# arkworks-rs/ripp

Hardware: AMD Instinct MI355X
Metric: SIPP prover pairing-products/sec at n=2^20 BLS12-381 (higher is better)
Workload: dtype u32

## Files before the change

### ripp_amd/csrc/engine.hip

```cpp
#include <hip/hip_runtime.h>
#include <atomic>
#include <csignal>
#include <sched.h>
#include <condition_variable>
#include <deque>
#include <functional>
#include <memory>
#include <future>
#include <chrono>
#include <cmath>
#include <cstdio>
#include <cstring>
#include <cstdlib>
#include <mutex>
#include <string>
#include <thread>
#include <vector>
#ifndef RIPP_BUILD_STAMP
#define RIPP_BUILD_STAMP __DATE__ " " __TIME__
#endif
#include "../../include/ripp_hip.h"
#include "kernels.hpp"
#include "line_products.hpp"
#include "msm.hpp"
// ... 36 lines not shown
        auto task = std::make_shared<std::packaged_task<decltype(f())()>>(std::forward<F>(f));
        auto fut = task->get_future();
        push([task]() { (*task)(); });
        return fut;
    }
    void set_hot(bool h) { hot_.store(h, std::memory_order_release); }
    template <class F> void parallel(int n, F&& fn) {
        if (n <= 0) return;
        std::atomic<int> left{n - 1};
        for (int t = 1; t < n; ++t) push([&fn, &left, t]() { fn(t); left.fetch_sub(1, std::memory_order_release); });
        fn(0);
        while (left.load(std::memory_order_acquire) > 0) RIPP_CPU_RELAX();
    }
private:
    void push(std::function<void()> job) {
        { std::lock_guard<std::mutex> lk(mu_); q_.emplace_back(std::move(job)); }
        pending_.fetch_add(1, std::memory_order_release);
        if (sleepers_.load(std::memory_order_acquire) > 0) cv_.notify_one();
    }
    void run() {
        for (;;) {
            std::function<void()> job;
            const auto t0 = std::chrono::steady_clock::now();
            for (int spin = 0; hot_.load(std::memory_order_acquire) && pending_.load(std::memory_order_acquire) == 0; ++spin) {
                RIPP_CPU_RELAX();
                if ((spin & 1023) == 1023 && std::chrono::steady_clock::now() - t0 > std::chrono::milliseconds(50)) break;
            }
            {
                std::unique_lock<std::mutex> lk(mu_);
                if (q_.empty()) { sleepers_.fetch_add(1); cv_.wait(lk, [this]() { return stop_ || !q_.empty(); }); sleepers_.fetch_sub(1); }
                if (stop_ && q_.empty()) return;
                job = std::move(q_.front()); q_.pop_front();
                pending_.fetch_sub(1, std::memory_order_release);
            }
            job();
        }
    }
    std::vector<std::thread> th_; std::deque<std::function<void()>> q_; std::mutex mu_; std::condition_variable cv_; bool stop_ = false;
    std::atomic<int> pending_{0}, sleepers_{0}; std::atomic<bool> hot_{false};
};
static int effective_cpus();
HostPool& host_pool() {
    static HostPool pool([]() -> unsigned { if (const char* s = std::getenv("RIPP_HOST_WORKERS")) { const int v = std::atoi(s); if (v >= 1 && v <= 64) return (unsigned)v; } return effective_cpus() >= 14 ? 11u : 6u; }());
    return pool;
}
static int effective_cpus() {
    static const int n = []() {
        int c = (int)std::thread::hardware_concurrency();
        cpu_set_t set; CPU_ZERO(&set);
        if (sched_getaffinity(0, sizeof set, &set) == 0) { const int a = CPU_COUNT(&set); if (a > 0) c = a; }
        if (FILE* f = std::fopen("/sys/fs/cgroup/cpu.max", "r")) {
            char q[32] = {0}; long period = 0;
            if (std::fscanf(f, "%31s %ld", q, &period) == 2 && period > 0 && q[0] != 'm') { const long quota = std::atol(q); if (quota > 0) c = std::min<long>(c, (quota + period - 1) / period); }
            std::fclose(f);
        }
        return std::max(1, c);
    }();
    return n;
}
static bool hot_workers_pay(int ranks_on_node) { return effective_cpus() / std::max(1, ranks_on_node) >= 8; }
double now_ms(); bool trace_on();
void pairing_values(const Fp12* rows, int count, Fp12* out, int parts = 0) {
    if (parts <= 0) parts = host_pool().size() >= 11 ? (count >= 2 ? 5 : 8) : (count >= 2 ? 3 : 4);
    struct Seg { int k, hi, lo; };
    std::vector<Seg> segs;
    for (int k = 0; k < count; ++k) for (int g = 0; g < parts; ++g) segs.push_back({k, 62 - (63 * g) / parts, 62 - (63 * (g + 1)) / parts + 1});
    std::vector<Fp12> E(segs.size());
    auto work = [&rows, &segs, &E](size_t t) { const Seg& sg = segs[t]; E[t] = final_exponentiation(miller_combine_range(rows + (size_t)sg.k * N_LINES, sg.hi, sg.lo)); };
    const double tp0 = now_ms();
    host_pool().parallel((int)segs.size(), [&work](int t) { work((size_t)t); });
    const double tp1 = now_ms();
    host_pool().parallel(count, [&](int k) {
        Fp12 c = E[(size_t)k * parts];
        for (int g = 1; g < parts; ++g) { const Seg& sg = segs[(size_t)k * parts + g]; for (int b = sg.hi; b >= sg.lo; --b) c = cyclotomic_sqr(c); c = mul(c, E[(size_t)k * parts + g]); }
        out[k] = BLS_X_NEG ? conj(c) : c; });
    if (trace_on()) fprintf(stderr, "[ripp] pairing_values(%d x %d): ranges %.3f ms, join %.3f ms\n", count, parts, tp1 - tp0, now_ms() - tp1);
}
struct Engine;
Engine* g_engine = nullptr;
std::atomic<int> g_live_handles{0};

#define HIPCHK(expr) do { hipError_t e_ = (expr); if (e_ != hipSuccess) { set_err(std::string(#expr) + ": " + hipGetErrorString(e_)); return RIPP_ERR_DEVICE; } } while (0)
void set_err(const std::string& s) { g_err = s; }
bool trace_on();
double now_ms() { return std::chrono::duration<double, std::milli>(std::chrono::steady_clock::now().time_since_epoch()).count(); }

inline unsigned nblk(size_t n, unsigned b) { return (unsigned)((n + b - 1) / b); }
inline uint32_t pow2_floor(uint32_t v) { uint32_t p = 1; while ((p << 1) <= v && (p << 1) != 0) p <<= 1; return p; }

std::atomic<size_t> g_dev_bytes{0};
std::atomic<uint64_t> g_call_epoch{1};
struct Engine;
thread_local Engine* t_engine = nullptr;
size_t evict_idle_scratch(Engine* e);
struct DevBuf {
    void* p = nullptr; size_t cap = 0; uint64_t epoch = 0;
    int32_t reserve(size_t bytes) {
        epoch = g_call_epoch.load(std::memory_order_relaxed);
        if (bytes <= cap) return RIPP_OK;
        release();
        hipError_t err = hipMalloc(&p, bytes);
        if (err == hipErrorOutOfMemory && t_engine) {
            (void)hipGetLastError();
            const size_t freed = evict_idle_scratch(t_engine);
            if (trace_on()) fprintf(stderr, "[ripp] out of device memory for %zu bytes: %zu bytes of idle scratch freed, retrying\n", bytes, freed);
            err = freed ? hipMalloc(&p, bytes) : err;
        }
        if (err != hipSuccess) { p = nullptr; (void)hipGetLastError(); set_err(std::string("hipMalloc(&p, bytes): ") + hipGetErrorString(err) + " (" + std::to_string(bytes) + " bytes wanted, " + std::to_string(g_dev_bytes.load()) + " held by the library)"); return RIPP_ERR_DEVICE; }
        cap = bytes; g_dev_bytes.fetch_add(bytes, std::memory_order_relaxed); return RIPP_OK;
    }
    void release() { if (p) { (void)hipFree(p); g_dev_bytes.fetch_sub(cap, std::memory_order_relaxed); } p = nullptr; cap = 0; }
    template <class T> T* as() { return reinterpret_cast<T*>(p); }
};

struct PinBuf {
    void* p = nullptr; size_t cap = 0; hipEvent_t ev = nullptr; bool pending = false;
    bool blocking = false;
    bool ev_blocking = false;
    int32_t wait() { if (pending) { HIPCHK(hipEventSynchronize(ev)); pending = false; } return RIPP_OK; }
    int32_t reserve(size_t bytes) {
        int32_t rc = wait(); if (rc) return rc;
        if (ev && ev_blocking != blocking) { (void)hipEventDestroy(ev); ev = nullptr; }
        if (!ev) { HIPCHK(hipEventCreateWithFlags(&ev, hipEventDisableTiming | (blocking ? hipEventBlockingSync : 0))); ev_blocking = blocking; }
        if (bytes <= cap) return RIPP_OK;
        if (p) { (void)hipHostFree(p); p = nullptr; cap = 0; }
        HIPCHK(hipHostMalloc(&p, bytes, hipHostMallocDefault)); cap = bytes; return RIPP_OK;
    }
    int32_t send(void* dst, size_t bytes, hipStream_t st) {
        HIPCHK(hipMemcpyAsync(dst, p, bytes, hipMemcpyHostToDevice, st)); HIPCHK(hipEventRecord(ev, st)); pending = true; return RIPP_OK;
    }
    void release() { if (pending && ev) (void)hipEventSynchronize(ev); pending = false; if (p) (void)hipHostFree(p); p = nullptr; cap = 0; if (ev) (void)hipEventDestroy(ev); ev = nullptr; }
    template <class T> T* as() { return reinterpret_cast<T*>(p); }
};

struct MsmScratch {
    DevBuf digits, hist, offs, cursor, slotoffs, spw, sorted, slots, buckets, seg, seg2, win, out;
    DevBuf ext;
    DevBuf flags;
    DevBuf nflag;
    void* host_out = nullptr;
    void release() { for (DevBuf* b : {&digits, &hist, &offs, &cursor, &slotoffs, &spw, &sorted, &slots, &buckets, &seg, &seg2, &win, &out, &ext, &flags, &nflag}) b->release(); if (host_out) (void)hipHostFree(host_out); host_out = nullptr; }
};

struct Timer {
    hipEvent_t a{}, b{};
    int32_t init() { HIPCHK(hipEventCreate(&a)); HIPCHK(hipEventCreate(&b)); return RIPP_OK; }
    void destroy() { if (a) (void)hipEventDestroy(a); if (b) (void)hipEventDestroy(b); a = b = nullptr; }
};

struct Engine {
    int device = -1;
    hipStream_t stream = nullptr, stream2 = nullptr;
    hipEvent_t ev_fork = nullptr, ev_join = nullptr, ev_join3 = nullptr;
    hipEvent_t ev_t0 = nullptr, ev_t1 = nullptr;
    int n_simd = 1024;
    DevBuf lines, partA, partB, jacG1, jacG2, tmpA, tmpB, tmpR, affG1, affG2;
    DevBuf qtab;
    MsmScratch msm_scratch[2];
    DevBuf kzg_q[2];
    PinBuf stage[4];
    DevBuf kzg_bases[2];
    hipStream_t stream3 = nullptr;
    hipStream_t stream4 = nullptr;
    hipEvent_t ev_join4 = nullptr;
    DevBuf fold_tab1, fold_mult, fold_tab, fold_jac1, fold_jac2;
    DevBuf fix_flags, scale_flags;
    const void* tab_owner = nullptr;
    struct JobBufCache { DevBuf d[15]; PinBuf p[4]; bool full = false; void release() { for (DevBuf& b : d) b.release(); for (PinBuf& b : p) b.release(); full = false; } } job_cache;
    size_t msm_chunk_min = (size_t)1 << 20;
    size_t msm_lds_sort_min = 0;
    const void* g2tab_hi = nullptr; size_t g2tab_half = 0;
    size_t vm_scale_max = (size_t)1 << 14;
    size_t vm_joint_max = (size_t)1 << 13;
    size_t lp_fq_min = 0;
    size_t ml_fq_min = 0;
    size_t fq_min_g1 = (size_t)1 << 12;
    size_t fq_min = (size_t)1 << 15;
    size_t fold_tab_min = 32768;
    size_t msm_vm_merge_max = 16384;
    hipStream_t stream5 = nullptr;
    hipEvent_t ev_join5 = nullptr;
    Fp12* pinned_rows = nullptr;
    size_t pinned_rows_cap = 0;
    std::vector<std::pair<hipEvent_t, hipEvent_t>> ev_lines, ev_prod;
    std::vector<std::pair<hipEvent_t, hipEvent_t>> ev_fold_async;
    size_t tail_pipe_max = (size_t)1 << 11;
    size_t vm_tree_max = (size_t)1 << 16;
    size_t vm_fold_max = (size_t)1 << 11;
    DevBuf vm_flag;
    size_t vm_lines_max = (size_t)1 << 15;
    size_t gls_split_max = (size_t)1 << 14;
    size_t max_pairs_per_batch = (size_t)1 << 19;
    size_t mem_cap = 0;
    int mem_tier = 0;
    bool mem_fits(size_t need, size_t held) const {
        if (need <= held) return true;
        const size_t extra = need - held;
        if (mem_cap) return g_dev_bytes.load(std::memory_order_relaxed) + extra <= mem_cap;
        size_t fr = 0, tot = 0;
        if (hipMemGetInfo(&fr, &tot) != hipSuccess) return true;
        return extra + std::max<size_t>((size_t)2 << 30, tot / 50) <= fr;
    }
    size_t pairs_cap(size_t want) {
        want = std::max<size_t>(1, std::min(want, max_pairs_per_batch));
        const size_t per = (size_t)N_LINES * LINE_CHUNKS * sizeof(uint4);
        auto bytes = [per](size_t pairs) { return ((pairs + 63) & ~(size_t)63) * per + (size_t)MAX_PRODUCTS * 64 * per; };
        if (bytes(want) <= lines.cap) return want;
        size_t w = want;
        while (w > 4096 && !mem_fits(bytes(w), lines.cap)) w = (w + 1) / 2;
        if (w < want) mem_tier |= 8;
        return w;
    }
    ripp_stats stats{};
    std::vector<Engine*> peers; bool virtual_devices = false;
    Engine* aux = nullptr;
    Engine* aux_engine() {
        if (!aux) { Engine* a = new Engine(); if (a->init(device) != RIPP_OK) { delete a; return nullptr; } aux = a; }
        aux->refresh_switches(); aux->stats = ripp_stats{};
        return aux;
    }
    struct Switches { bool no_vm = false, no_precompute = false, no_fold_tables = false, no_msm_glv = false, lp_one_lane = false, no_endo = false, no_fq = false, no_xscale = false, no_share = false, no_fuse = false, no_prebuild = false, fuse_tables = false, no_job_cache = false, no_lp_kara = false; } sw;
    struct Sizes { size_t vm_lines_max, vm_fold_max, vm_tree_max, gls_split_max, msm_vm_merge_max, fold_tab_min, fq_min, lp_fq_min, vm_joint_max, vm_scale_max, tail_pipe_max, ml_fq_min, fq_min_g1, msm_lds_sort_min, msm_chunk_min; } defaults{};
    MsmTune msm_tune;
    double cal_ms_per_pair = 0, cal_hash_bytes_per_ms = 0;
    int look_eighths = -1; double ranks_per_device = 1.0; bool look_static = false, quiet_waits_cfg = false, agg_sequential = false, scale_no_fq = false;
    int hot_workers_cfg = 0;
    uint32_t comm_timeout_ms = 0, plan_derate_pct = 0, n_devices_cfg = 0;
    void refresh_switches() {
        msm_tune = MsmTune();
        vm_lines_max = defaults.vm_lines_max; vm_fold_max = defaults.vm_fold_max; vm_tree_max = defaults.vm_tree_max; gls_split_max = defaults.gls_split_max;
        msm_vm_merge_max = defaults.msm_vm_merge_max; fold_tab_min = defaults.fold_tab_min; fq_min = defaults.fq_min; lp_fq_min = defaults.lp_fq_min; vm_joint_max = defaults.vm_joint_max;
        vm_scale_max = defaults.vm_scale_max; tail_pipe_max = defaults.tail_pipe_max; ml_fq_min = defaults.ml_fq_min; fq_min_g1 = defaults.fq_min_g1; msm_lds_sort_min = defaults.msm_lds_sort_min; msm_chunk_min = defaults.msm_chunk_min;
        sw = Switches(); look_eighths = -1; ranks_per_device = 1.0; look_static = quiet_waits_cfg = agg_sequential = scale_no_fq = false; mem_cap = 0; hot_workers_cfg = 0; comm_timeout_ms = plan_derate_pct = n_devices_cfg = 0;
        if (g_cfg_set) {
            const ripp_config& c = g_cfg;
            sw.no_vm = c.no_vm; sw.no_precompute = c.no_precompute; sw.no_fold_tables = c.no_fold_tables; sw.no_msm_glv = c.no_msm_glv; sw.lp_one_lane = c.lp_one_lane;
            sw.no_endo = c.no_endo; sw.no_fq = c.no_fq; sw.no_xscale = c.no_xscale; sw.no_share = c.no_share; sw.no_fuse = c.no_fuse; sw.fuse_tables = c.fuse_tables; scale_no_fq = c.scale_no_fq; agg_sequential = c.agg_sequential; look_static = c.look_static; quiet_waits_cfg = c.quiet_waits;
            look_eighths = c.look_eighths; ranks_per_device = c.ranks_per_device > 1 ? (double)c.ranks_per_device : 1.0;
            msm_tune.c = c.msm_c; msm_tune.ch = c.msm_ch; msm_tune.gmin = c.msm_gmin; sw.no_prebuild = c.no_prebuild;
            mem_cap = (size_t)c.mem_cap_bytes; hot_workers_cfg = (int)c.hot_workers; sw.no_job_cache = c.no_job_cache != 0;
            sw.no_lp_kara = c.no_lp_karatsuba != 0; comm_timeout_ms = c.comm_timeout_ms; plan_derate_pct = c.plan_derate_pct; n_devices_cfg = c.n_devices;
            vm_lines_max = c.vm_lines_max; vm_fold_max = c.vm_fold_max; vm_tree_max = c.vm_tree_max; gls_split_max = c.gls_split_max; msm_vm_merge_max = c.msm_vm_merge_max; fold_tab_min = c.fold_tab_min;
            fq_min = c.fq_min; lp_fq_min = c.lp_fq_min; vm_joint_max = c.vm_joint_max; vm_scale_max = c.vm_scale_max; tail_pipe_max = c.tail_pipe_max; ml_fq_min = c.ml_fq_min; fq_min_g1 = c.fq_min_g1; msm_lds_sort_min = c.msm_lds_sort_min; msm_chunk_min = c.msm_chunk_min;
        }
        { const char* s; if ((s = std::getenv("RIPP_MSM_C"))) msm_tune.c = std::atoi(s); if ((s = std::getenv("RIPP_MSM_CH"))) msm_tune.ch = (uint32_t)std::strtoul(s, nullptr, 10); if ((s = std::getenv("RIPP_MSM_GMIN"))) msm_tune.gmin = (uint32_t)std::strtoul(s, nullptr, 10); }
        auto env_sz = [](const char* k, size_t& v) { if (const char* s = std::getenv(k)) v = (size_t)std::strtoull(s, nullptr, 10); };
        env_sz("RIPP_VM_LINES_MAX", vm_lines_max); env_sz("RIPP_VM_FOLD_MAX", vm_fold_max); env_sz("RIPP_VM_TREE_MAX", vm_tree_max);
        env_sz("RIPP_GLS_SPLIT_MAX", gls_split_max); env_sz("RIPP_MSM_VM_MERGE_MAX", msm_vm_merge_max); env_sz("RIPP_FOLD_TAB_MIN", fold_tab_min);
        env_sz("RIPP_FQ_MIN", fq_min); env_sz("RIPP_LP_FQ_MIN", lp_fq_min); env_sz("RIPP_VM_JOINT_MAX", vm_joint_max);
        env_sz("RIPP_MSM_LDS_SORT_MIN", msm_lds_sort_min); env_sz("RIPP_MSM_CHUNK_MIN", msm_chunk_min);
        env_sz("RIPP_VM_SCALE_MAX", vm_scale_max); env_sz("RIPP_TAIL_PIPE_MAX", tail_pipe_max); env_sz("RIPP_ML_FQ_MIN", ml_fq_min); env_sz("RIPP_FQ_MIN_G1", fq_min_g1);
        auto env_on = [](const char* k, bool& v) { if (std::getenv(k)) v = true; };
        env_on("RIPP_NO_VM", sw.no_vm); env_on("RIPP_NO_PRECOMPUTE", sw.no_precompute); env_on("RIPP_NO_FOLD_TABLES", sw.no_fold_tables); env_on("RIPP_NO_MSM_GLV", sw.no_msm_glv);
        env_on("RIPP_LP_ONE_LANE", sw.lp_one_lane);
        env_on("RIPP_NO_ENDO", sw.no_endo);
        env_on("RIPP_NO_XSCALE", sw.no_xscale);
        env_on("RIPP_NO_LP_KARA", sw.no_lp_kara);
        env_on("RIPP_NO_FQ", sw.no_fq);
        env_on("RIPP_FUSE_TABLES", sw.fuse_tables);
        env_on("RIPP_NO_JOB_CACHE", sw.no_job_cache);
        env_sz("RIPP_MEM_CAP_BYTES", mem_cap);
        if (const char* s = std::getenv("RIPP_HOT_WORKERS")) hot_workers_cfg = std::atoi(s) ? 1 : 2;
        { auto env_u32 = [](const char* k, uint32_t& v) { if (const char* s = std::getenv(k)) v = (uint32_t)std::strtoul(s, nullptr, 10); };
          env_u32("RIPP_COMM_TIMEOUT_MS", comm_timeout_ms); env_u32("RIPP_PLAN_DERATE_PCT", plan_derate_pct); env_u32("RIPP_N_DEVICES", n_devices_cfg);
          virtual_devices = false; if (const char* s = std::getenv("RIPP_VIRTUAL_DEVICES")) { n_devices_cfg = (uint32_t)std::strtoul(s, nullptr, 10); virtual_devices = true; } }
        env_on("RIPP_NO_PREBUILD", sw.no_prebuild);
        env_on("RIPP_NO_FUSE", sw.no_fuse);
        env_on("RIPP_NO_SHARE", sw.no_share);
        env_on("RIPP_SCALE_NO_FQ", scale_no_fq); env_on("RIPP_AGG_SEQUENTIAL", agg_sequential); env_on("RIPP_LOOK_STATIC", look_static); env_on("RIPP_QUIET_WAITS", quiet_waits_cfg);
        if (const char* s = std::getenv("RIPP_LOOK_ITEMS")) look_eighths = 8 * std::max(0, std::atoi(s));
        if (const char* s = std::getenv("RIPP_LOOK_EIGHTHS")) look_eighths = std::max(0, std::atoi(s));
        if (const char* s = std::getenv("RIPP_RANKS_PER_DEVICE")) ranks_per_device = std::max(1.0, std::atof(s));
#if !defined(RIPP_AB_KERNELS) || defined(RIPP_BLS12_377)
        sw.lp_one_lane = false;
#endif
    }

    int32_t init(int dev) {
        int n = 0;
        if (hipGetDeviceCount(&n) != hipSuccess || n <= 0) { set_err("no HIP device available (libripp_hip has no CPU fallback)"); return RIPP_ERR_DEVICE; }
        if (dev < 0 || dev >= n) { set_err("device ordinal out of range"); return RIPP_ERR_ARG; }
        HIPCHK(hipSetDevice(dev));
        HIPCHK(hipStreamCreateWithFlags(&stream, hipStreamNonBlocking));
        HIPCHK(hipStreamCreateWithFlags(&stream2, hipStreamNonBlocking));
        HIPCHK(hipStreamCreateWithFlags(&stream3, hipStreamNonBlocking));
        HIPCHK(hipStreamCreateWithFlags(&stream4, hipStreamNonBlocking)); HIPCHK(hipEventCreateWithFlags(&ev_join4, hipEventDisableTiming));
        HIPCHK(hipStreamCreateWithFlags(&stream5, hipStreamNonBlocking)); HIPCHK(hipEventCreateWithFlags(&ev_join5, hipEventDisableTiming));
        HIPCHK(hipEventCreateWithFlags(&ev_fork, hipEventDisableTiming)); HIPCHK(hipEventCreateWithFlags(&ev_join, hipEventDisableTiming)); HIPCHK(hipEventCreateWithFlags(&ev_join3, hipEventDisableTiming));
        HIPCHK(hipEventCreate(&ev_t0)); HIPCHK(hipEventCreate(&ev_t1));
        { hipDeviceProp_t pr; if (hipGetDeviceProperties(&pr, dev) == hipSuccess) n_simd = pr.multiProcessorCount * 4; }
        defaults = Sizes{vm_lines_max, vm_fold_max, vm_tree_max, gls_split_max, msm_vm_merge_max, fold_tab_min, fq_min, lp_fq_min, vm_joint_max, vm_scale_max, tail_pipe_max, ml_fq_min, fq_min_g1, msm_lds_sort_min, msm_chunk_min};
        refresh_switches();
        device = dev;
        return RIPP_OK;
    }
    void destroy() {
        if (aux) { aux->destroy(); delete aux; aux = nullptr; }
        for (Engine* p : peers) { (void)hipSetDevice(p->device); p->destroy(); delete p; }
        if (!peers.empty()) { peers.clear(); (void)hipSetDevice(device); }
        for (DevBuf* b : {&lines, &partA, &partB, &jacG1, &jacG2, &tmpA, &tmpB, &tmpR, &affG1, &affG2, &qtab, &vm_flag, &scale_tab, &fold_tab1, &fold_mult, &fold_tab, &fold_jac1, &fold_jac2, &fix_flags, &scale_flags}) b->release();
        msm_scratch[0].release(); msm_scratch[1].release(); kzg_q[0].release(); kzg_q[1].release(); kzg_bases[0].release(); kzg_bases[1].release(); job_cache.release();
        if (stream3) (void)hipStreamDestroy(stream3);
        if (stream4) (void)hipStreamDestroy(stream4); if (ev_join4) (void)hipEventDestroy(ev_join4);
        if (stream5) (void)hipStreamDestroy(stream5); if (ev_join5) (void)hipEventDestroy(ev_join5);
        if (pinned_rows) (void)hipHostFree(pinned_rows);
        for (PinBuf& b : stage) b.release();
        for (auto& e : ev_lines) { (void)hipEventDestroy(e.first); (void)hipEventDestroy(e.second); }
        for (auto& e : ev_prod) { (void)hipEventDestroy(e.first); (void)hipEventDestroy(e.second); }
        for (auto& e : ev_fold_async) { (void)hipEventDestroy(e.first); (void)hipEventDestroy(e.second); }
        if (stream) (void)hipStreamDestroy(stream);
        if (stream2) (void)hipStreamDestroy(stream2);
        if (ev_fork) (void)hipEventDestroy(ev_fork); if (ev_join) (void)hipEventDestroy(ev_join); if (ev_join3) (void)hipEventDestroy(ev_join3);
        if (ev_t0) (void)hipEventDestroy(ev_t0); if (ev_t1) (void)hipEventDestroy(ev_t1);
        if (ev_quiet) (void)hipEventDestroy(ev_quiet);
    }
    int32_t ensure_pinned_rows(size_t rows) {
        if (rows <= pinned_rows_cap) return RIPP_OK;
        if (pinned_rows) (void)hipHostFree(pinned_rows);
        HIPCHK(hipHostMalloc((void**)&pinned_rows, rows * sizeof(Fp12), hipHostMallocDefault));
        pinned_rows_cap = rows; return RIPP_OK;
    }
    bool quiet_waits = false; hipEvent_t ev_quiet = nullptr;
    int32_t sync() {
        if (quiet_waits) {
            if (!ev_quiet) HIPCHK(hipEventCreateWithFlags(&ev_quiet, hipEventDisableTiming | hipEventBlockingSync));
            HIPCHK(hipEventRecord(ev_quiet, stream)); HIPCHK(hipEventSynchronize(ev_quiet)); return RIPP_OK;
        }
        HIPCHK(hipStreamSynchronize(stream)); return RIPP_OK;
    }

    int32_t mark(std::vector<std::pair<hipEvent_t, hipEvent_t>>& v, bool begin) {
        if (begin) { hipEvent_t a, b; HIPCHK(hipEventCreate(&a)); HIPCHK(hipEventCreate(&b)); v.emplace_back(a, b); HIPCHK(hipEventRecord(a, stream)); }
        else HIPCHK(hipEventRecord(v.back().second, stream));
        return RIPP_OK;
    }
    void collect_kernel_stats() {
        auto drain = [](std::vector<std::pair<hipEvent_t, hipEvent_t>>& v, double& sum, uint64_t& cnt) {
            for (auto& e : v) { float ms = 0; if (hipEventElapsedTime(&ms, e.first, e.second) == hipSuccess) { sum += ms; ++cnt; } (void)hipEventDestroy(e.first); (void)hipEventDestroy(e.second); }
            v.clear(); };
        drain(ev_lines, stats.kernel_miller_lines_ms_sum, stats.kernel_miller_lines_launches);
        drain(ev_prod, stats.kernel_line_products_ms_sum, stats.kernel_line_products_launches);
        uint64_t nf = 0; drain(ev_fold_async, stats.fold_ms, nf);
    }

    DevBuf scale_tab;
    int32_t scale_g1_dev(const G1A* base, uint32_t base_stride, const Fr* k, size_t n, G1J* out, hipStream_t st = nullptr) {
        if (n == 0) return RIPP_OK;
        if (!st) st = stream;
        if (sw.no_endo) {
            hipLaunchKernelGGL(HIP_KERNEL_NAME(k_scale_pts<Fp>), dim3(nblk(n, 256)), dim3(256), 0, st, base, base_stride, k, (uint32_t)n, out);
            HIPCHK(hipGetLastError());
            return RIPP_OK;
        }
        if (n <= vm_scale_max && !sw.no_vm) {
            hipLaunchKernelGGL(k_vm_scale_g1, dim3(nblk(n, 4 * VM_EPW)), dim3(256), 4 * VM_EPW * VM_SCALE_SLOTS * sizeof(VmSlot), st, base, base_stride, k, (uint32_t)n, out);
            HIPCHK(hipGetLastError());
            return RIPP_OK;
        }
        int32_t rc = scale_tab.reserve((size_t)SCALE_TAB * G1J_CHUNKS * n * sizeof(uint4)); if (rc) return rc;
        if (!sw.no_fq && !scale_no_fq)
        {
            if ((rc = scale_flags.reserve(n + 16))) return rc;
            hipLaunchKernelGGL(k_scale_g1_glv_q, dim3(nblk(n, 256)), dim3(256), 0, st, base, base_stride, k, (uint32_t)n, scale_tab.as<uint4>(), out, scale_flags.as<uint8_t>());
            hipLaunchKernelGGL(k_scale_g1_fix, dim3(FIX_GRID), dim3(64), 0, st, base, base_stride, k, (uint32_t)n, out, scale_flags.as<uint8_t>());
        }
        else
        hipLaunchKernelGGL(k_scale_g1_glv, dim3(nblk(n, 256)), dim3(256), 0, st, base, base_stride, k, (uint32_t)n, scale_tab.as<uint4>(), out);
        HIPCHK(hipGetLastError());
        return RIPP_OK;
    }

    template <class F> int32_t normalize_dev(const Jac<F>* in, size_t n, Affine<F>* out, hipStream_t st = nullptr) {
        if (n == 0) return RIPP_OK;
        if (!st) st = stream;
        uint32_t K = (uint32_t)std::min<size_t>(16, std::max<size_t>(1, n / 65536));
        uint32_t T = (uint32_t)((n + K - 1) / K);
        hipLaunchKernelGGL(HIP_KERNEL_NAME(k_normalize<F>), dim3(nblk(T, 256)), dim3(256), 0, st, in, (uint32_t)n, out, T);
        HIPCHK(hipGetLastError());
        return RIPP_OK;
    }


    template <class F> int32_t msm_launch(MsmScratch& ms, hipStream_t st, const Affine<F>* bases, const Fr* scalars, size_t n, const std::function<int32_t()>* bases_arrive = nullptr) {
        if (!ms.host_out) HIPCHK(hipHostMalloc(&ms.host_out, sizeof(G2J), hipHostMallocDefault));
        if (n == 0) { *reinterpret_cast<Jac<F>*>(ms.host_out) = jac_inf<F>(); return bases_arrive ? (*bases_arrive)() : RIPP_OK; }
        const bool no_glv = sw.no_msm_glv;
        const size_t nreal = n;
        const MsmPlan p = msm_plan(nreal, no_glv ? 1 : std::is_same<F, Fp>::value ? 2 : 4, msm_tune);
        n = p.n;
        const size_t nwb = (size_t)p.nwin * p.nb;
        const uint32_t max_slots = (uint32_t)(n / p.ch + std::min<size_t>(p.nb, n) + 1);
        uint32_t nseg = (p.nb + p.seg - 1) / p.seg;
        int32_t rc;
        if ((rc = ms.digits.reserve((size_t)p.nwin * n * sizeof(uint16_t))) || (rc = ms.hist.reserve(nwb * 4)) || (rc = ms.offs.reserve(nwb * 4)) ||
            (rc = ms.cursor.reserve(nwb * 4)) || (rc = ms.slotoffs.reserve(nwb * 4)) || (rc = ms.spw.reserve(p.nwin * 4)) ||
            (rc = ms.sorted.reserve((size_t)p.nwin * n * 4)) || (rc = ms.slots.reserve((size_t)p.nwin * max_slots * sizeof(Jac<F>))) ||
            (rc = ms.buckets.reserve(nwb * sizeof(Jac<F>))) || (rc = ms.seg.reserve((size_t)p.nwin * nseg * sizeof(Jac<F>))) ||
            (rc = ms.seg2.reserve((size_t)p.nwin * ((nseg + MSM_SEG_FAN - 1) / MSM_SEG_FAN) * sizeof(Jac<F>))) ||
            (rc = ms.win.reserve(64 * sizeof(Jac<F>))) || (rc = ms.out.reserve(sizeof(Jac<F>)))) return rc;
        HIPCHK(hipMemsetAsync(ms.hist.p, 0, nwb * 4, st));
        const bool lds_sort = n >= msm_lds_sort_min && p.nb <= 8192;
        const uint32_t tile = msm_sort_tile(p);
        hipLaunchKernelGGL(k_msm_digits, dim3(nblk(nreal, 256)), dim3(256), 0, st, scalars, p, ms.digits.as<uint16_t>(), lds_sort ? nullptr : ms.hist.as<uint32_t>());
        if (lds_sort) hipLaunchKernelGGL(k_msm_hist_lds, dim3(nblk(n, tile), p.nwin), dim3(MSM_SORT_BLOCK), 0, st, ms.digits.as<uint16_t>(), p, tile, ms.hist.as<uint32_t>());
        hipLaunchKernelGGL(k_msm_scan, dim3(p.nwin), dim3(1024), 0, st, ms.hist.as<uint32_t>(), p, ms.offs.as<uint32_t>(), ms.cursor.as<uint32_t>(), ms.slotoffs.as<uint32_t>(), ms.spw.as<uint32_t>());
        if (lds_sort) hipLaunchKernelGGL(k_msm_scatter_lds, dim3(nblk(n, tile), p.nwin), dim3(MSM_SORT_BLOCK), 0, st, ms.digits.as<uint16_t>(), p, tile, ms.cursor.as<uint32_t>(), ms.sorted.as<uint32_t>());
        else hipLaunchKernelGGL(k_msm_scatter, dim3(nblk(n, 256)), dim3(256), 0, st, ms.digits.as<uint16_t>(), p, ms.cursor.as<uint32_t>(), ms.sorted.as<uint32_t>());
        if (bases_arrive && (rc = (*bases_arrive)())) return rc;
        const bool hom = !sw.no_vm;
        const size_t vm_lds = 4 * VM_EPW * VmCurve<F>::SLOTS * sizeof(VmSlot);
        if (!sw.no_fq) {
            const int split = (int)(n / nreal);
            if ((rc = ms.ext.reserve(n * sizeof(Affine<F>))) || (rc = ms.flags.reserve((size_t)p.nwin * max_slots + 16))) return rc;
            hipLaunchKernelGGL(HIP_KERNEL_NAME(k_msm_extend_q<F>), dim3(nblk(nreal, 256), split), dim3(256), 0, st, bases, (uint32_t)nreal, split, ms.ext.as<QAff<F>>());
            hipLaunchKernelGGL(HIP_KERNEL_NAME(k_msm_slot_sum_q<F>), dim3(nblk(max_slots, 64), p.nwin), dim3(64), 0, st, ms.ext.as<QAff<F>>(), p, ms.hist.as<uint32_t>(), ms.offs.as<uint32_t>(),
                               ms.slotoffs.as<uint32_t>(), ms.spw.as<uint32_t>(), ms.sorted.as<uint32_t>(), ms.slots.as<Jac<F>>(), max_slots, hom, ms.flags.as<uint8_t>());
            if (hom) {
                if ((rc = ms.nflag.reserve(16))) return rc;
                if (trace_on()) HIPCHK(hipMemsetAsync(ms.nflag.p, 0, 4, st));
                hipLaunchKernelGGL(HIP_KERNEL_NAME(k_msm_slot_sum_fix_vm<F>), dim3(FIX_GRID), dim3(64), VM_EPW * VmCurve<F>::SLOTS * sizeof(VmSlot), st, bases, p, ms.hist.as<uint32_t>(), ms.offs.as<uint32_t>(),
                                   ms.slotoffs.as<uint32_t>(), ms.spw.as<uint32_t>(), ms.sorted.as<uint32_t>(), ms.slots.as<Jac<F>>(), max_slots, ms.flags.as<uint8_t>(), trace_on() ? ms.nflag.as<uint32_t>() : nullptr);
                if (trace_on()) {
                    uint32_t nf = 0; HIPCHK(hipMemcpyAsync(&nf, ms.nflag.p, 4, hipMemcpyDeviceToHost, st)); HIPCHK(hipStreamSynchronize(st));
                    fprintf(stderr, "[ripp] msm %s n=%zu: %u of %u slots had an exceptional addition (redone on the field VM)\n", std::is_same<F, Fp>::value ? "G1" : "G2", nreal, nf, (uint32_t)p.nwin * max_slots);
                }
            } else
            hipLaunchKernelGGL(HIP_KERNEL_NAME(k_msm_slot_sum_fix<F>), dim3(FIX_GRID), dim3(64), 0, st, bases, p, ms.hist.as<uint32_t>(), ms.offs.as<uint32_t>(),
                               ms.slotoffs.as<uint32_t>(), ms.spw.as<uint32_t>(), ms.sorted.as<uint32_t>(), ms.slots.as<Jac<F>>(), max_slots, hom, ms.flags.as<uint8_t>());
        } else
        hipLaunchKernelGGL(HIP_KERNEL_NAME(k_msm_slot_sum<F>), dim3(nblk(max_slots, 64), p.nwin), dim3(64), 0, st, bases, p, ms.hist.as<uint32_t>(), ms.offs.as<uint32_t>(),
                           ms.slotoffs.as<uint32_t>(), ms.spw.as<uint32_t>(), ms.sorted.as<uint32_t>(), ms.slots.as<Jac<F>>(), max_slots, hom);
        uint32_t passes = 0;
        for (uint32_t stride = 1; passes < (uint32_t)MSM_GROUP_PASSES && n / p.ch + 1 > (size_t)p.gmin * stride; stride *= MSM_SLOT_GROUP, ++passes)
            hipLaunchKernelGGL(HIP_KERNEL_NAME(k_msm_slot_group<F>), dim3(nblk(max_slots, 64), p.nwin), dim3(64), 0, st, p, ms.hist.as<uint32_t>(),
                               ms.slotoffs.as<uint32_t>(), ms.spw.as<uint32_t>(), ms.slots.as<Jac<F>>(), max_slots, stride, hom);
        if (hom && nwb <= msm_vm_merge_max)
            hipLaunchKernelGGL(HIP_KERNEL_NAME(k_msm_vm_merge<F>), dim3(nblk(p.nb, 4 * VM_EPW), p.nwin), dim3(256), vm_lds, st, p, ms.hist.as<uint32_t>(), ms.slotoffs.as<uint32_t>(),
                               ms.slots.as<Jac<F>>(), max_slots, ms.buckets.as<Jac<F>>(), passes);
        else
            hipLaunchKernelGGL(HIP_KERNEL_NAME(k_msm_bucket_merge<F>), dim3(nblk(p.nb, 64), p.nwin), dim3(64), 0, st, p, ms.hist.as<uint32_t>(), ms.slotoffs.as<uint32_t>(),
                               ms.slots.as<Jac<F>>(), max_slots, ms.buckets.as<Jac<F>>(), passes, hom);
        Jac<F>* cur = ms.seg.as<Jac<F>>(); Jac<F>* nxt = ms.seg2.as<Jac<F>>();
        if (hom) {
            hipLaunchKernelGGL(HIP_KERNEL_NAME(k_msm_vm_segments<F>), dim3(nblk(nseg, 4 * VM_EPW), p.nwin), dim3(256), vm_lds, st, p, ms.buckets.as<Jac<F>>(), cur, nseg);
            while (nseg > 1) {
                const uint32_t nout = (nseg + MSM_SEG_FAN - 1) / MSM_SEG_FAN;
                hipLaunchKernelGGL(HIP_KERNEL_NAME(k_msm_vm_reduce<F>), dim3(nblk(nout, 4 * VM_EPW), p.nwin), dim3(256), vm_lds, st, cur, nseg, nxt, nout);
                std::swap(cur, nxt); nseg = nout;
            }
            hipLaunchKernelGGL(HIP_KERNEL_NAME(k_msm_finish_vm<F>), dim3(1), dim3(64), VM_EPW * VmCurve<F>::SLOTS * sizeof(VmSlot), st, p, cur, ms.win.as<Jac<F>>(), ms.out.as<Jac<F>>());
        } else {
            hipLaunchKernelGGL(HIP_KERNEL_NAME(k_msm_segments<F>), dim3(nblk(nseg, 64), p.nwin), dim3(64), 0, st, p, ms.buckets.as<Jac<F>>(), cur, nseg);
            while (nseg > (uint32_t)MSM_SEG_FAN) {
                const uint32_t nout = (nseg + MSM_SEG_FAN - 1) / MSM_SEG_FAN;
                hipLaunchKernelGGL(HIP_KERNEL_NAME(k_msm_seg_reduce<F>), dim3(nblk(nout, 64), p.nwin), dim3(64), 0, st, cur, nseg, nxt, nout);
                std::swap(cur, nxt); nseg = nout;
            }
            hipLaunchKernelGGL(HIP_KERNEL_NAME(k_msm_finish<F>), dim3(1), dim3(64), 0, st, p, cur, nseg, ms.win.as<Jac<F>>(), ms.out.as<Jac<F>>());
        }
        HIPCHK(hipGetLastError());
        HIPCHK(hipMemcpyAsync(ms.host_out, ms.out.p, sizeof(Jac<F>), hipMemcpyDeviceToHost, st));
        return RIPP_OK;
    }
    template <class F> int32_t msm_dev(const Affine<F>* bases, const Fr* scalars, size_t n, Jac<F>* out_host, const std::function<int32_t()>* bases_arrive = nullptr) {
        int32_t rc = msm_launch<F>(msm_scratch[0], stream, bases, scalars, n, bases_arrive); if (rc) return rc;
// ... 20 lines not shown
                    else { cs.b[ng] = ps.b[p]; cs.first[ng] = (uint8_t)p; cs.np[ng] = 1; ++ng; }
                }
                hipLaunchKernelGGL(k_miller_lines_q, dim3(nblk(m, 256), ng), dim3(256), 0, stream, cs, (uint32_t)m, lines.as<uint4>(), stride);
                stats.chains_lines += m * (size_t)ng;
            } else
                hipLaunchKernelGGL(k_miller_lines, dim3(nblk(m, 256), nprod), dim3(256), 0, stream, ps, (uint32_t)m, lines.as<uint4>(), stride);
            HIPCHK(hipGetLastError());
            if ((rc = mark(ev_lines, false)) != RIPP_OK) return rc;
            stats.pairs_lines += m * nprod;
        }
        int pieces[8] = {nprod, 0, 0, 0, 0, 0, 0, 0};
        if (nprod > 8) {
            static const int fill[8] = {30, 15, 10, 6, 5, 3, 2, 1};
            int left = nprod, k = 0;
            while (left > 0 && k < 8) { int f = 0; while (fill[f] > left) ++f; pieces[k++] = fill[f]; left -= fill[f]; }
            if (left > 0) pieces[7] += left;
        }
        else if (m * (size_t)nprod >= ((size_t)1 << 17) && !sw.lp_one_lane) {
            if (nprod == 8) { pieces[0] = 6; pieces[1] = 2; } else if (nprod == 7) { pieces[0] = 5; pieces[1] = 2; } else if (nprod == 4) { pieces[0] = 2; pieces[1] = 2; }
        }
        int p_lo = 0;
        for (int pc = 0; pc < 8 && pieces[pc] > 0; p_lo += pieces[pc], ++pc)
            if ((rc = enqueue_stage2(p_lo, pieces[pc], m, stride, dst_pinned)) != RIPP_OK) return rc;
        return RIPP_OK;
    }
    int32_t enqueue_stage2(int p_lo, int np2, size_t m, size_t stride, Fp12* dst_pinned) {
        int32_t rc;
        const size_t nrows = (size_t)np2 * N_LINES;
        const uint4* lrows = lines.as<uint4>() + (size_t)p_lo * N_LINES * LINE_CHUNKS * stride;
#if !defined(RIPP_BLS12_377)
        const bool lp_kara = !sw.no_fq && !sw.no_lp_kara && !sw.lp_one_lane && m * (size_t)np2 >= lp_fq_min;
#else
        const bool lp_kara = false;
#endif
        const uint32_t per_wave = sw.lp_one_lane ? 64 : lp_kara ? LK_GROUPS_PER_WAVE : LP_GROUPS_PER_WAVE;
        uint32_t T = (uint32_t)std::max<size_t>(per_wave, ((size_t)n_simd * RIPP_OCC_PROD / nrows) * per_wave);
        if (T > m) T = (uint32_t)m;
        if ((rc = partA.reserve(nrows * FP12_CHUNKS * (size_t)T * sizeof(uint4))) != RIPP_OK) return rc;
        if ((rc = partB.reserve(nrows * FP12_CHUNKS * (size_t)((T + 1) / 2) * sizeof(uint4))) != RIPP_OK) return rc;
        if ((rc = mark(ev_prod, true)) != RIPP_OK) return rc;
#if defined(RIPP_AB_KERNELS) && !defined(RIPP_BLS12_377)
        if (sw.lp_one_lane)
            hipLaunchKernelGGL(k_line_products1, dim3(nblk(T, 64), (unsigned)nrows), dim3(64), 0, stream, lrows, stride, (uint32_t)m, partA.as<uint4>(), T);
        else
#endif
#if !defined(RIPP_BLS12_377)
        if (lp_kara)
            hipLaunchKernelGGL(k_line_products_k, dim3(nblk(T, LK_GROUPS_PER_WAVE), (unsigned)nrows), dim3(64), 0, stream, lrows, stride, (uint32_t)m, partA.as<uint4>(), T);
        else
#endif
        if (!sw.no_fq && m * (size_t)np2 >= lp_fq_min)
            hipLaunchKernelGGL(k_line_products_q, dim3(nblk(T, LP_GROUPS_PER_WAVE), (unsigned)nrows), dim3(64), 0, stream, lrows, stride, (uint32_t)m, partA.as<uint4>(), T);
        else
            hipLaunchKernelGGL(k_line_products, dim3(nblk(T, LP_GROUPS_PER_WAVE), (unsigned)nrows), dim3(64), 0, stream, lrows, stride, (uint32_t)m, partA.as<uint4>(), T);
        HIPCHK(hipGetLastError());
        if ((rc = mark(ev_prod, false)) != RIPP_OK) return rc;
        stats.pairs_products += m * (size_t)np2;
        uint4* cur = partA.as<uint4>(); uint4* nxt = partB.as<uint4>();
        while (T > 1) {
            const int R = ((size_t)T * nrows > (size_t)n_simd * 64) ? 4 : 2;
            const uint32_t Tout = (T + R - 1) / R;
            if (R == 2 && (size_t)Tout * nrows <= vm_tree_max && !sw.no_vm)
                hipLaunchKernelGGL(k_vm_fp12_tree, dim3(nblk(Tout, 2 * VM_EPW), (unsigned)nrows), dim3(128), 2 * VM_EPW * VM_F12_SLOTS * sizeof(VmSlot), stream, cur, T, nxt, Tout);
            else
            hipLaunchKernelGGL(k_fp12_tree, dim3(nblk(Tout, 64), (unsigned)nrows), dim3(64), 0, stream, cur, T, nxt, Tout, R);
            HIPCHK(hipGetLastError());
            std::swap(cur, nxt); T = Tout;
        }
        HIPCHK(hipMemcpyAsync(dst_pinned + (size_t)p_lo * N_LINES, cur, nrows * sizeof(Fp12), hipMemcpyDeviceToHost, stream));
        return RIPP_OK;
    }
    int32_t step_products(const G1A* const* a, const G2A* const* b, int nprod, size_t M, Fp12* rows_out) {
        const size_t nrows = (size_t)nprod * N_LINES;
        for (size_t r = 0; r < nrows; ++r) rows_out[r] = Fp12::one();
        if (M == 0) return RIPP_OK;
        int32_t rc;
        if ((rc = ensure_pinned_rows(nrows)) != RIPP_OK) return rc;
        if (nprod > MAX_PRODUCTS) return RIPP_ERR_ARG;
        const size_t batch = std::min(M, std::max<size_t>(1, pairs_cap(std::min(max_pairs_per_batch, M * (size_t)nprod)) / nprod));
        for (size_t off = 0; off < M; off += batch) {
            const size_t m = std::min(batch, M - off);
            if ((rc = enqueue_products(a, b, nprod, off, m, pinned_rows)) != RIPP_OK) return rc;
            if ((rc = sync()) != RIPP_OK) return rc;
            for (size_t r = 0; r < nrows; ++r) rows_out[r] = (off == 0) ? pinned_rows[r] : mul(rows_out[r], pinned_rows[r]);
        }
        return RIPP_OK;
    }
};

int32_t get_engine(Engine** out) {
    if (!g_engine) {
        Engine* e = new Engine();
        int32_t rc = e->init(0);
        if (rc != RIPP_OK) { delete e; return rc; }
        g_engine = e;
    }
    if (hipSetDevice(g_engine->device) != hipSuccess) { set_err("hipSetDevice failed"); return RIPP_ERR_DEVICE; }
    g_engine->refresh_switches();
    g_call_epoch.fetch_add(1, std::memory_order_relaxed); t_engine = g_engine;
    *out = g_engine; return RIPP_OK;
}

bool trace_on() { static const bool on = std::getenv("RIPP_TRACE") != nullptr; return on; }
size_t evict_idle_scratch(Engine* e) {
    const uint64_t now = g_call_epoch.load(std::memory_order_relaxed);
    (void)hipDeviceSynchronize();
    const size_t before = g_dev_bytes.load();
    bool tables = false;
    for (DevBuf* b : {&e->lines, &e->partA, &e->partB, &e->qtab, &e->scale_tab, &e->jacG1, &e->jacG2, &e->affG1, &e->affG2, &e->tmpA, &e->tmpB, &e->tmpR}) if (b->p && b->epoch != now) b->release();
    for (DevBuf* b : {&e->fold_tab1, &e->fold_mult, &e->fold_tab, &e->fold_jac1, &e->fold_jac2}) if (b->p && b->epoch != now) { b->release(); tables = true; }
    if (tables) { e->tab_owner = nullptr; e->g2tab_hi = nullptr; }
    for (int k = 0; k < 2; ++k) {
        MsmScratch& ms = e->msm_scratch[k];
        for (DevBuf* b : {&ms.digits, &ms.hist, &ms.offs, &ms.cursor, &ms.slotoffs, &ms.spw, &ms.sorted, &ms.slots, &ms.buckets, &ms.seg, &ms.seg2, &ms.win, &ms.ext, &ms.flags}) if (b->p && b->epoch != now) b->release();
        for (DevBuf* b : {&e->kzg_q[k], &e->kzg_bases[k]}) if (b->p && b->epoch != now) b->release();
    }
    if (e->job_cache.full) e->job_cache.release();
    const size_t after = g_dev_bytes.load();
    return before > after ? before - after : 0;
}

ScalarBits scalar_bits(const Fr& s_mont) {
    const Fr c = from_mont(s_mont);
    ScalarBits sb; int top = -1;
    for (int i = 0; i < 8; ++i) { sb.w[i] = c.l[i]; }
    for (int i = 255; i >= 0; --i) if ((c.l[i >> 5] >> (i & 31)) & 1u) { top = i; break; }
    sb.nbits = top + 1; return sb;
}

int naf_recode(const uint32_t* words, int nwords, int8_t* digits, int maxd) {
    uint32_t w[10] = {0};
    for (int i = 0; i < nwords; ++i) w[i] = words[i];
    auto is_zero = [&]() { for (int i = 0; i <= nwords; ++i) if (w[i]) return false; return true; };
    int n = 0;
    while (!is_zero() && n < maxd) {
        int8_t d = 0;
        if (w[0] & 1u) {
            d = (int8_t)(2 - (int)(w[0] & 3u));
            if (d > 0) { w[0] &= ~1u; }
            else { for (int i = 0; i <= nwords; ++i) { if (++w[i] != 0) break; } }
        }
        digits[n++] = d;
        for (int i = 0; i < nwords; ++i) w[i] = (w[i] >> 1) | (w[i + 1] << 31);
        w[nwords] >>= 1;
    }
    return n;
}
NafDigits naf_digits(const Fr& s_mont) {
    const Fr c = from_mont(s_mont);
    NafDigits nd; std::memset(&nd, 0, sizeof nd);
    nd.len = naf_recode(c.l, 8, nd.d, 258);
    return nd;
}
GlsDigits gls_digits(const Fr& s_mont) {
    const Fr c = from_mont(s_mont);
    uint64_t v[4] = {(uint64_t)c.l[0] | ((uint64_t)c.l[1] << 32), (uint64_t)c.l[2] | ((uint64_t)c.l[3] << 32),
                     (uint64_t)c.l[4] | ((uint64_t)c.l[5] << 32), (uint64_t)c.l[6] | ((uint64_t)c.l[7] << 32)};
    GlsDigits g; std::memset(&g, 0, sizeof g);
    int maxlen = 0;
    for (int j = 0; j < 4; ++j) {
        unsigned __int128 rem = 0;
        for (int i = 3; i >= 0; --i) { const unsigned __int128 cur = (rem << 64) | v[i]; v[i] = (uint64_t)(cur / BLS_X_ABS); rem = cur % BLS_X_ABS; }
        const uint64_t dj = (uint64_t)rem;
        const uint32_t words[2] = {(uint32_t)dj, (uint32_t)(dj >> 32)};
        const int len = naf_recode(words, 2, g.d[j], 66);
        if (len > maxlen) maxlen = len;
    }
    g.len = maxlen;
    return g;
}

void glv_split(const Fr& s_mont, uint32_t rem[9], uint32_t quo[8]) {
    const Fr c = from_mont(s_mont);
    const uint32_t lam[8] = RIPP_GLV_LAMBDA;
    for (int i = 0; i < 9; ++i) rem[i] = 0; for (int i = 0; i < 8; ++i) quo[i] = 0;
    for (int bit = 255; bit >= 0; --bit) {
        for (int i = 8; i > 0; --i) rem[i] = (rem[i] << 1) | (rem[i - 1] >> 31);
        rem[0] = (rem[0] << 1) | ((c.l[bit >> 5] >> (bit & 31)) & 1u);
        bool ge = rem[8] != 0;
        if (!ge) { ge = true; for (int i = 7; i >= 0; --i) { if (rem[i] != lam[i]) { ge = rem[i] > lam[i]; break; } } }
        if (ge) { uint32_t borrow = 0; for (int i = 0; i < 8; ++i) rem[i] = subb32(rem[i], lam[i], borrow); rem[8] -= borrow; quo[bit >> 5] |= 1u << (bit & 31); }
    }
}
GlvDigits glv_digits(const Fr& s_mont) {
    uint32_t rem[9], quo[8]; glv_split(s_mont, rem, quo);
    GlvDigits g; std::memset(&g, 0, sizeof g);
    const int l1 = naf_recode(rem, 5, g.d1, 131), l2 = naf_recode(quo, 5, g.d2, 131);
    g.len = l1 > l2 ? l1 : l2;
    return g;
}

int wnaf4_recode(uint64_t v, int8_t* digits, int maxd, int W = RIPP_FOLD_W) {
    unsigned __int128 k = v; int len = 0;
    while (k != 0 && len < maxd) {
        int d = 0;
        if ((uint64_t)k & 1u) { d = (int)((uint64_t)k & ((1u << W) - 1)); if (d >= (1 << (W - 1))) d -= 1 << W; if (d >= 0) k -= (unsigned)d; else k += (unsigned)(-d); }
        digits[len++] = (int8_t)d;
        k >>= 1;
    }
    return len;
}
Wnaf4 split32_wnaf(const Fr& s_mont, int W = RIPP_FOLD_W) {
    const Fr c = from_mont(s_mont);
    Wnaf4 g; std::memset(&g, 0, sizeof g);
    for (int t = 0; t < 4; ++t) g.len = std::max(g.len, wnaf4_recode(c.l[t], g.d[t], 35, W));
    return g;
}
int tab_width(int M) { int w = 2; while ((1 << (w - 2)) < M) ++w; return w; }
void glv_split(const Fr& s_mont, uint32_t rem[9], uint32_t quo[8]);
WnafG1x4 fused_digits_g1(const Fr& x0, const Fr& x1, int W) {
    WnafG1x4 g; std::memset(&g, 0, sizeof g);
    const Fr c0 = from_mont(x0), c1 = from_mont(x1);
    uint32_t rem[9], quo[8]; glv_split(mul(x0, x1), rem, quo);
    const uint32_t* src[4] = {c0.l, rem, quo, c1.l};
    for (int u = 0; u < 4; ++u) for (int b = 0; b < 4; ++b) g.len = std::max(g.len, wnaf4_recode(src[u][b], g.d[4 * u + b], 35, W));
    return g;
}
GlvDigits split64_digits(const Fr& s_mont) {
    const Fr c = from_mont(s_mont);
    GlvDigits g; std::memset(&g, 0, sizeof g);
    const int l1 = naf_recode(&c.l[0], 2, g.d1, 131), l2 = naf_recode(&c.l[2], 2, g.d2, 131);
    g.len = l1 > l2 ? l1 : l2;
    return g;
}
bool fits_128(const Fr& s_mont) { const Fr c = from_mont(s_mont); return (c.l[4] | c.l[5] | c.l[6] | c.l[7]) == 0; }
Gls8Digits gls8_digits(const Fr& s_mont) {
    const Fr c = from_mont(s_mont);
    uint64_t v[4] = {(uint64_t)c.l[0] | ((uint64_t)c.l[1] << 32), (uint64_t)c.l[2] | ((uint64_t)c.l[3] << 32),
                     (uint64_t)c.l[4] | ((uint64_t)c.l[5] << 32), (uint64_t)c.l[6] | ((uint64_t)c.l[7] << 32)};
    Gls8Digits g; std::memset(&g, 0, sizeof g);
    int maxlen = 0;
    for (int j = 0; j < 4; ++j) {
        unsigned __int128 rem = 0;
        for (int i = 3; i >= 0; --i) { const unsigned __int128 cur = (rem << 64) | v[i]; v[i] = (uint64_t)(cur / BLS_X_ABS); rem = cur % BLS_X_ABS; }
        const uint64_t dj = (uint64_t)rem;
        const uint32_t lo = (uint32_t)dj, hi = (uint32_t)(dj >> 32);
        const int l1 = naf_recode(&lo, 1, g.d[j], 35), l2 = naf_recode(&hi, 1, g.d[4 + j], 35);
        maxlen = std::max(maxlen, std::max(l1, l2));
    }
    g.len = maxlen;
    return g;
}

Wnaf16 gls16_wnaf(const Fr& s_mont, int W = RIPP_FOLD_W) {
    const Fr c = from_mont(s_mont);
    uint64_t v[4] = {(uint64_t)c.l[0] | ((uint64_t)c.l[1] << 32), (uint64_t)c.l[2] | ((uint64_t)c.l[3] << 32),
                     (uint64_t)c.l[4] | ((uint64_t)c.l[5] << 32), (uint64_t)c.l[6] | ((uint64_t)c.l[7] << 32)};
    Wnaf16 g; std::memset(&g, 0, sizeof g);
    for (int j = 0; j < 4; ++j) {
        unsigned __int128 rem = 0;
        for (int i = 3; i >= 0; --i) { const unsigned __int128 cur = (rem << 64) | v[i]; v[i] = (uint64_t)(cur / BLS_X_ABS); rem = cur % BLS_X_ABS; }
        const uint64_t dj = (uint64_t)rem;
        for (int b = 0; b < 4; ++b) g.len = std::max(g.len, wnaf4_recode((dj >> (16 * b)) & 0xffffu, g.d[4 * b + j], 19, W));
    }
    return g;
}
Wnaf16x3 fused_digits_g2(const Fr& x0, const Fr& x1, int W) {
    Wnaf16x3 g; g.s[0] = gls16_wnaf(mul(x0, x1), W); g.s[1] = gls16_wnaf(x0, W); g.s[2] = gls16_wnaf(x1, W);
    g.len = std::max(g.s[0].len, std::max(g.s[1].len, g.s[2].len));
    return g;
}

GlsDigits gls_wnaf(const Fr& s_mont, int W) {
    const Fr c = from_mont(s_mont);
    uint64_t v[4] = {(uint64_t)c.l[0] | ((uint64_t)c.l[1] << 32), (uint64_t)c.l[2] | ((uint64_t)c.l[3] << 32),
                     (uint64_t)c.l[4] | ((uint64_t)c.l[5] << 32), (uint64_t)c.l[6] | ((uint64_t)c.l[7] << 32)};
    GlsDigits g; std::memset(&g, 0, sizeof g);
    for (int j = 0; j < 4; ++j) {
        unsigned __int128 rem = 0;
        for (int i = 3; i >= 0; --i) { const unsigned __int128 cur = (rem << 64) | v[i]; v[i] = (uint64_t)(cur / BLS_X_ABS); rem = cur % BLS_X_ABS; }
        g.len = std::max(g.len, wnaf4_recode((uint64_t)rem, g.d[j], 66, W));
    }
    return g;
}

SplitDigits split_digits_g1(const Fr& s_mont) {
    const GlvDigits g = split64_digits(s_mont);
    SplitDigits d; std::memset(&d, 0, sizeof d);
    for (int i = 0; i < g.len && i < 68; ++i) { d.d[0][i] = g.d1[i]; d.d[1][i] = g.d2[i]; }
    d.len = g.len; return d;
}
SplitDigits split_digits_g2(const Fr& s_mont) {
    const Gls8Digits g = gls8_digits(s_mont);
    SplitDigits d; std::memset(&d, 0, sizeof d);
    for (int t = 0; t < 8; ++t) for (int i = 0; i < g.len; ++i) d.d[t][i] = g.d[t][i];
    d.len = g.len; return d;
}

SplitDigits split_digits_g1_glv(const Fr& s_mont) {
    uint32_t rem[9], quo[8]; glv_split(s_mont, rem, quo);
    SplitDigits d; std::memset(&d, 0, sizeof d);
    const int l0 = naf_recode(&rem[0], 2, d.d[0], 67), l1 = naf_recode(&quo[0], 2, d.d[1], 67), l2 = naf_recode(&rem[2], 2, d.d[2], 67), l3 = naf_recode(&quo[2], 2, d.d[3], 67);
    d.len = std::max(std::max(l0, l1), std::max(l2, l3)); return d;
}

template <class T> int32_t upload(Engine* e, DevBuf& buf, const void* host, size_t n, T** dev) {
    int32_t rc = buf.reserve(std::max<size_t>(n, 1) * sizeof(T)); if (rc != RIPP_OK) return rc;
    if (n) HIPCHK(hipMemcpyAsync(buf.p, host, n * sizeof(T), hipMemcpyHostToDevice, e->stream));
    *dev = buf.as<T>(); return RIPP_OK;
}


double g_digest_hash_ms = 0, g_digest_wait_ms = 0;
void statement_digest(const G1A* a, const G2A* b, const Fr* r, size_t n, const Fp12& value, uint8_t digest[32], std::atomic<uint64_t>* progress = nullptr) {
    fs::Blake2s h;
    g_digest_hash_ms = g_digest_wait_ms = 0;
    const uint64_t len = (uint64_t)n;
    constexpr size_t BLK = 1 << 13; constexpr int RING = 6;
    const size_t item[3] = {96, 192, 32};
    struct Seg { int kind; size_t s, e; };
    std::vector<Seg> segs;
    for (int kind = 0; kind < 3; ++kind) for (size_t s0 = 0; s0 < n; s0 += BLK) segs.push_back({kind, s0, std::min(n, s0 + BLK)});
    struct Ring { std::vector<uint8_t> b[RING]; };
    static std::mutex pool_mu; static std::vector<std::unique_ptr<Ring>> pool;
    std::unique_ptr<Ring> ring;
    { std::lock_guard<std::mutex> lk(pool_mu); if (!pool.empty()) { ring = std::move(pool.back()); pool.pop_back(); } }
    if (!ring) { ring.reset(new Ring()); for (auto& v : ring->b) v.resize(BLK * 192); }
    struct Return { std::unique_ptr<Ring>& r; std::mutex& m; std::vector<std::unique_ptr<Ring>>& p; ~Return() { std::lock_guard<std::mutex> lk(m); p.emplace_back(std::move(r)); } } give_back{ring, pool_mu, pool};
    std::vector<uint8_t>* const buf = ring->b;
    std::vector<std::future<void>> fut(segs.size());
    auto launch = [&](size_t j) {
        const Seg sg = segs[j]; uint8_t* out = buf[j % RING].data();
        fut[j] = host_pool().submit([a, b, r, sg, out]() {
            for (size_t i = sg.s; i < sg.e; ++i) {
                if (sg.kind == 0) fs::ser_g1(a[i], out + (i - sg.s) * 96);
                else if (sg.kind == 1) fs::ser_g2(b[i], out + (i - sg.s) * 192);
                else fs::ser_fr(r[i], out + (i - sg.s) * 32);
            } });
    };
    for (size_t j = 0; j < segs.size() && j < (size_t)RING - 1; ++j) launch(j);
    int cur_kind = -1;
    for (size_t j = 0; j < segs.size(); ++j) {
        if (segs[j].kind != cur_kind) {
            for (int k = cur_kind + 1; k <= segs[j].kind; ++k) h.update(reinterpret_cast<const uint8_t*>(&len), 8);
            cur_kind = segs[j].kind;
        }
        const double t0 = now_ms();
        fut[j].get();
        const double t1 = now_ms();
        h.update(buf[j % RING].data(), (segs[j].e - segs[j].s) * item[segs[j].kind]);
        if (progress) progress->fetch_add((segs[j].e - segs[j].s) * item[segs[j].kind], std::memory_order_relaxed);
        g_digest_wait_ms += t1 - t0; g_digest_hash_ms += now_ms() - t1;
        if (j + RING - 1 < segs.size()) launch(j + RING - 1);
    }
    for (int k = cur_kind + 1; k < 3; ++k) h.update(reinterpret_cast<const uint8_t*>(&len), 8);
    uint8_t gt[576]; fs::ser_gt(value, gt); h.update(gt, 576);
    h.finish(digest);
}

}

struct ripp_sipp_job {
    size_t n_local = 0, len = 0;
    int rank = 0, world = 1, world0 = 1;
    DevBuf a0, b0, r0;
    DevBuf a, b, a_next, b_next, jac1, jac2;
    size_t tab2_stride = 0; bool tab_ready = false;
    size_t tab_cnt = 0; int tab_M = FOLD_TAB_M; bool tab_fused = false;
    Fr bs = Fr::one(); bool bs_on = false; bool tab_on_lo = false; bool xs_enabled = false;
    DevBuf a_pow, b_pow; bool pre_ready = false;
    struct LookItem {
        int R = 0, side = 0, level = 0;
        size_t npairs = 0, q = 0;
        std::vector<Fp12> Z;
        std::vector<std::future<Fp12>> fe, pend;
    };
    std::vector<LookItem> look; PinBuf look_rows[2];
    double look_deadline = 0;
    std::atomic<uint64_t> hash_done{0}; uint64_t hash_total = 0; double hash_t0 = 0;
    bool no_window = false;
    size_t hash_n = 0;
    DevBuf a_pow_h, b_pow_h, parts1, parts2; bool pre_vm_ready = false, pre_vm_side = false;
    PinBuf tp_rows[2]; size_t tp_round[2] = {~(size_t)0, ~(size_t)0};
    std::vector<G1A> ha; std::vector<G2A> hb; std::vector<Fr> hr;
    const G1A* ha_ext = nullptr; const G2A* hb_ext = nullptr; const Fr* hr_ext = nullptr;
    bool hash_prestarted = false;
    fs::FiatShamirRng rng; bool seeded = false;
    std::thread hash_thread; uint8_t digest[32]; std::atomic<bool> digest_ready{false};
    double t_begin = 0;
};

namespace {

int32_t job_begin(Engine* e, ripp_sipp_job* j) {
    const size_t n = j->n_local;
    int32_t rc;
    if ((rc = j->a.reserve(n * sizeof(G1A))) != RIPP_OK) return rc;
    if ((rc = j->b.reserve(n * sizeof(G2A))) != RIPP_OK) return rc;
    if ((rc = j->a_next.reserve(std::max<size_t>(n / 2, 1) * sizeof(G1A))) != RIPP_OK) return rc;
    if ((rc = j->b_next.reserve(std::max<size_t>(n / 2, 1) * sizeof(G2A))) != RIPP_OK) return rc;
    if ((rc = j->jac1.reserve(n * sizeof(G1J))) != RIPP_OK) return rc;
    if ((rc = j->jac2.reserve(std::max<size_t>(n / 2, 1) * sizeof(G2J))) != RIPP_OK) return rc;
    e->stats = ripp_stats{};
    j->t_begin = now_ms();
    hipEvent_t t0 = e->ev_t0, t1 = e->ev_t1;
    HIPCHK(hipEventRecord(t0, e->stream));
    if ((rc = e->scale_g1_dev(j->a0.as<G1A>(), 1u, j->r0.as<Fr>(), n, j->jac1.as<G1J>())) != RIPP_OK) return rc;
    if ((rc = e->normalize_dev<Fp>(j->jac1.as<G1J>(), n, j->a.as<G1A>())) != RIPP_OK) return rc;
    HIPCHK(hipMemcpyAsync(j->b.p, j->b0.p, n * sizeof(G2A), hipMemcpyDeviceToDevice, e->stream));
    HIPCHK(hipEventRecord(t1, e->stream));
    if ((rc = e->sync()) != RIPP_OK) return rc;
    float ms = 0; (void)hipEventElapsedTime(&ms, t0, t1); e->stats.scale_ms += ms;
    j->len = n; j->seeded = false; j->world = j->world0;
    j->bs = Fr::one(); j->bs_on = false;
    j->pre_vm_ready = false; j->pre_vm_side = false; j->pre_ready = false; j->look.clear(); j->tp_round[0] = j->tp_round[1] = ~(size_t)0;
    return RIPP_OK;
}

int32_t job_round_partials(Engine* e, ripp_sipp_job* j, Fp12* rows ) {
    const size_t half = j->len / 2;
    const G1A* a = j->a.as<G1A>(); const G2A* b = j->b.as<G2A>();
    const G1A* as[2] = {a + half, a};
    const G2A* bs[2] = {b, b + half};
    const double t0 = now_ms();
    int32_t rc = e->step_products(as, bs, 2, half, rows);
    e->stats.miller_products_ms += now_ms() - t0;
    return rc;
}

bool fold_g2_table_pays(const Engine* e, size_t half) { return half >= e->fold_tab_min && half > e->gls_split_max && !e->sw.no_fold_tables; }
bool fold_g2_table_fits(const Engine* e, size_t half) {
    const size_t need = half * (5 * 4 * sizeof(G2A) + 3 * sizeof(G2J)) + 65536, held = e->fold_mult.cap + e->fold_tab.cap + e->fold_jac2.cap;
    return need <= held || e->mem_fits(need, held);
}
bool xscale_round(const Engine* e, const ripp_sipp_job* j, size_t half) {
    if (!j->xs_enabled || e->sw.no_endo || e->sw.no_xscale) return false;
    if (fold_g2_table_pays(e, half)) return true;
    return j->bs_on && half <= e->gls_split_max && 2 * half > e->vm_joint_max && half > e->vm_fold_max;
}
int32_t job_precompute_vm(Engine* e, ripp_sipp_job* j, bool side = false) {
    const size_t half = j->len / 2;
    if (half == 0 || half > e->vm_fold_max || e->sw.no_vm || e->sw.no_precompute) return RIPP_OK;
    int32_t rc;
    if ((rc = j->a_pow_h.reserve(half * sizeof(G1J))) || (rc = j->b_pow_h.reserve(half * sizeof(G2J))) || (rc = j->parts1.reserve(2 * half * sizeof(G1J))) || (rc = j->parts2.reserve(8 * half * sizeof(G2J)))) return rc;
    hipLaunchKernelGGL(HIP_KERNEL_NAME(k_vm_pow2<Fp>), dim3(nblk(half, 4 * VM_EPW)), dim3(256), 4 * VM_EPW * VmCurve<Fp>::SLOTS * sizeof(VmSlot), e->stream2, j->a.as<G1A>() + half, (uint32_t)half, 64, j->a_pow_h.as<G1J>());
    hipStream_t s2 = e->stream;
    if (side) { HIPCHK(hipStreamWaitEvent(e->stream3, e->ev_t1, 0)); s2 = e->stream3; }
    hipLaunchKernelGGL(HIP_KERNEL_NAME(k_vm_pow2<Fp2>), dim3(nblk(half, 4 * VM_EPW)), dim3(256), 4 * VM_EPW * VmCurve<Fp2>::SLOTS * sizeof(VmSlot), s2, j->b.as<G2A>() + half, (uint32_t)half, 32, j->b_pow_h.as<G2J>());
    HIPCHK(hipGetLastError());
    if (side) HIPCHK(hipEventRecord(e->ev_join3, e->stream3));
    j->pre_vm_side = side;
    j->pre_vm_ready = true;
    return RIPP_OK;
}

int32_t job_precompute_round0(Engine* e, ripp_sipp_job* j, bool fuse = false) {
    const size_t half = j->len / 2, q = j->len / 4;
    if (half < ((size_t)1 << 16) || j->digest_ready.load() || j->no_window || e->sw.no_precompute) return RIPP_OK;
    int32_t rc;
    bool tables = !e->sw.no_fold_tables;
    j->tab_ready = false; j->tab_fused = false;
    auto tab_bytes = [](size_t M, size_t cnt) { return cnt * (4 * M * (sizeof(G1A) + sizeof(G2A)) + 16 * M * sizeof(G2A) + (M - 1) * (sizeof(G1J) + sizeof(G2J)) + 4) + 65536; };
    const size_t tab_held = e->fold_tab1.cap + e->fold_mult.cap + e->fold_tab.cap + e->fold_jac1.cap + e->fold_jac2.cap + e->fix_flags.cap;
    size_t M_half = FOLD_TAB_M;
    if (tables) {
        const bool want_fuse = fuse && xscale_round(e, j, half) && !e->sw.no_fq && !e->sw.no_fuse && q >= e->fq_min;
        if (want_fuse && !e->mem_fits(tab_bytes(4, 3 * q), tab_held)) { fuse = false; e->mem_tier = std::max(e->mem_tier & 7, 1) | (e->mem_tier & 8); }
        if (!(want_fuse && fuse)) {
            if (!e->mem_fits(tab_bytes(M_half, half), tab_held)) { M_half = 4; e->mem_tier = std::max(e->mem_tier & 7, 1) | (e->mem_tier & 8); }
            if (!e->mem_fits(tab_bytes(M_half, half), tab_held)) { tables = false; e->mem_tier = std::max(e->mem_tier & 7, 2) | (e->mem_tier & 8); }
        }
        if (!tables) e->sw.no_fold_tables = true;
    }
    if (!tables && !e->mem_fits(half * (sizeof(G1A) + sizeof(G2A) + sizeof(G1J) + sizeof(G2J)), j->a_pow.cap + j->b_pow.cap + j->jac1.cap + j->jac2.cap)) {
        e->mem_tier = 3 | (e->mem_tier & 8);
        if (trace_on()) fprintf(stderr, "[ripp] round-0 precomputation skipped: the device is short of memory\n");
        return RIPP_OK;
    }
    if (trace_on() && (e->mem_tier & 7)) fprintf(stderr, "[ripp] round-0 tables: memory tier %d (%s)\n", e->mem_tier & 7, tables ? "half-vector tables" : "pre-doubled bases only");
    if ((rc = j->a_pow.reserve(half * sizeof(G1A))) || (rc = j->b_pow.reserve(half * sizeof(G2A))) || (rc = j->jac1.reserve(half * sizeof(G1J))) || (rc = j->jac2.reserve(half * sizeof(G2J)))) return rc;
    if (!tables) {
        if (!e->sw.no_fq) hipLaunchKernelGGL(k_pow2_mul_g1_q, dim3(nblk(half, 256)), dim3(256), 0, e->stream, j->a.as<G1A>() + half, (uint32_t)half, 64, j->jac1.as<G1J>());
        else hipLaunchKernelGGL(HIP_KERNEL_NAME(k_pow2_mul<Fp>), dim3(nblk(half, 256)), dim3(256), 0, e->stream, j->a.as<G1A>() + half, (uint32_t)half, 64, j->jac1.as<G1J>());
        HIPCHK(hipGetLastError());
        if ((rc = e->normalize_dev<Fp>(j->jac1.as<G1J>(), half, j->a_pow.as<G1A>()))) return rc;
        if (!e->sw.no_fq) hipLaunchKernelGGL(k_pow2_mul_g2_q, dim3(nblk(half, 64)), dim3(64), 0, e->stream, j->b.as<G2A>() + half, (uint32_t)half, 32, j->jac2.as<G2J>());
        else hipLaunchKernelGGL(HIP_KERNEL_NAME(k_pow2_mul<Fp2>), dim3(nblk(half, 256)), dim3(256), 0, e->stream, j->b.as<G2A>() + half, (uint32_t)half, 32, j->jac2.as<G2J>());
        HIPCHK(hipGetLastError());
        if ((rc = e->normalize_dev<Fp2>(j->jac2.as<G2J>(), half, j->b_pow.as<G2A>()))) return rc;
        j->pre_ready = true;
        return RIPP_OK;
    }
    j->tab_on_lo = xscale_round(e, j, half);
    fuse = fuse && j->tab_on_lo && !e->sw.no_fq && !e->sw.no_fuse && q >= e->fq_min;
    const size_t M = fuse ? 4 : M_half;
    const size_t cnt = fuse ? 3 * q : half;
    const size_t qstride = (cnt + 63) & ~(size_t)63;
    const size_t njt = (M - 1) * cnt;
    if ((rc = e->fold_tab1.reserve(4 * M * cnt * sizeof(G1A))) || (rc = e->fold_mult.reserve(4 * M * cnt * sizeof(G2A))) || (rc = e->fold_tab.reserve(16 * M * G2A_CHUNKS * qstride * sizeof(uint4))) ||
        (rc = e->fold_jac1.reserve(njt * sizeof(G1J))) || (rc = e->fold_jac2.reserve(njt * sizeof(G2J))) || (rc = e->fix_flags.reserve(4 * cnt + 16))) return rc;
    e->tab_owner = j;
    G1A* t1 = e->fold_tab1.as<G1A>(); G2A* t2 = e->fold_mult.as<G2A>();
    G1J* sj1 = e->fold_jac1.as<G1J>(); G2J* sj2 = e->fold_jac2.as<G2J>();
    HIPCHK(hipMemcpyAsync(t1, j->a.as<G1A>() + (fuse ? q : half), cnt * sizeof(G1A), hipMemcpyDeviceToDevice, e->stream));
    HIPCHK(hipMemcpyAsync(t2, j->b.as<G2A>() + (j->tab_on_lo ? 0 : half), cnt * sizeof(G2A), hipMemcpyDeviceToDevice, e->stream));
    for (int b = 0; b < 4; ++b) {
        G1A* base1 = t1 + M * b * cnt; G2A* base2 = t2 + M * b * cnt;
        if (b > 0) {
            if (!e->sw.no_fq) hipLaunchKernelGGL(k_pow2_mul_g1_q, dim3(nblk(cnt, 256)), dim3(256), 0, e->stream, base1 - M * cnt, (uint32_t)cnt, 32, sj1);
            else hipLaunchKernelGGL(HIP_KERNEL_NAME(k_pow2_mul<Fp>), dim3(nblk(cnt, 256)), dim3(256), 0, e->stream, base1 - M * cnt, (uint32_t)cnt, 32, sj1);
            HIPCHK(hipGetLastError());
            if ((rc = e->normalize_dev<Fp>(sj1, cnt, base1))) return rc;
            if (!e->sw.no_fq) hipLaunchKernelGGL(k_pow2_mul_g2_q, dim3(nblk(cnt, 64)), dim3(64), 0, e->stream, base2 - M * cnt, (uint32_t)cnt, 16, sj2);
            else hipLaunchKernelGGL(HIP_KERNEL_NAME(k_pow2_mul<Fp2>), dim3(nblk(cnt, 256)), dim3(256), 0, e->stream, base2 - M * cnt, (uint32_t)cnt, 16, sj2);
            HIPCHK(hipGetLastError());
            if ((rc = e->normalize_dev<Fp2>(sj2, cnt, base2))) return rc;
        }
        hipLaunchKernelGGL(HIP_KERNEL_NAME(k_odd_multiples<Fp>), dim3(nblk(cnt, 64)), dim3(64), 0, e->stream, base1, (uint32_t)cnt, (int)M, sj1);
        HIPCHK(hipGetLastError());
        if ((rc = e->normalize_dev<Fp>(sj1, njt, base1 + cnt))) return rc;
        if (!e->sw.no_fq) {
            hipLaunchKernelGGL(k_odd_multiples_q, dim3(nblk(cnt, 64)), dim3(64), 0, e->stream, base2, (uint32_t)cnt, (int)M, sj2, e->fix_flags.as<uint8_t>());
#if !defined(RIPP_INLINE_FALLBACK)
            hipLaunchKernelGGL(k_odd_multiples_fix, dim3(FIX_GRID), dim3(64), 0, e->stream, base2, (uint32_t)cnt, (int)M, sj2, e->fix_flags.as<uint8_t>());
#endif
        }
        else hipLaunchKernelGGL(HIP_KERNEL_NAME(k_odd_multiples<Fp2>), dim3(nblk(cnt, 64)), dim3(64), 0, e->stream, base2, (uint32_t)cnt, (int)M, sj2);
        HIPCHK(hipGetLastError());
        if ((rc = e->normalize_dev<Fp2>(sj2, njt, base2 + cnt))) return rc;
    }
    hipLaunchKernelGGL(k_g2_tab_images, dim3(nblk(cnt, 64), 4 * M), dim3(64), 0, e->stream, e->fold_mult.as<G2A>(), (uint32_t)cnt, (int)M, e->fold_tab.as<uint4>(), qstride);
    HIPCHK(hipGetLastError());
    j->tab2_stride = qstride; j->tab_cnt = cnt; j->tab_M = (int)M; j->tab_fused = fuse; j->tab_ready = true;
    return RIPP_OK;
}

int32_t fold_g2_table_build(Engine* e, hipStream_t st, const G2A* hi, size_t half) {
    constexpr int M = 4;
    const size_t qstride = (half + 63) & ~(size_t)63;
    int32_t rc;
    e->g2tab_hi = nullptr;
    if ((rc = e->fold_mult.reserve((size_t)M * half * sizeof(G2A))) || (rc = e->fold_tab.reserve((size_t)4 * M * G2A_CHUNKS * qstride * sizeof(uint4))) ||
        (rc = e->fold_jac2.reserve((size_t)(M - 1) * half * sizeof(G2J))) || (rc = e->fix_flags.reserve(4 * half + 16))) return rc;
    e->tab_owner = nullptr;
    G2A* mult = e->fold_mult.as<G2A>();
    HIPCHK(hipMemcpyAsync(mult, hi, half * sizeof(G2A), hipMemcpyDeviceToDevice, st));
    if (!e->sw.no_fq) {
        hipLaunchKernelGGL(k_odd_multiples_q, dim3(nblk(half, 64)), dim3(64), 0, st, hi, (uint32_t)half, M, e->fold_jac2.as<G2J>(), e->fix_flags.as<uint8_t>());
#if !defined(RIPP_INLINE_FALLBACK)
        hipLaunchKernelGGL(k_odd_multiples_fix, dim3(FIX_GRID), dim3(64), 0, st, hi, (uint32_t)half, M, e->fold_jac2.as<G2J>(), e->fix_flags.as<uint8_t>());
#endif
    }
    else hipLaunchKernelGGL(HIP_KERNEL_NAME(k_odd_multiples<Fp2>), dim3(nblk(half, 64)), dim3(64), 0, st, hi, (uint32_t)half, M, e->fold_jac2.as<G2J>());
    HIPCHK(hipGetLastError());
    if ((rc = e->normalize_dev<Fp2>(e->fold_jac2.as<G2J>(), (size_t)(M - 1) * half, mult + half, st)) != RIPP_OK) return rc;
    hipLaunchKernelGGL(k_g2_tab_images, dim3(nblk(half, 64), M), dim3(64), 0, st, mult, (uint32_t)half, M, e->fold_tab.as<uint4>(), qstride);
    HIPCHK(hipGetLastError());
    e->g2tab_hi = hi; e->g2tab_half = half;
    return RIPP_OK;
}
int32_t fold_g2_table(Engine* e, hipStream_t st, const G2A* hi, const G2A* lo, size_t half, const Fr& s, DevBuf& jac) {
    constexpr int M = 4;
    const size_t qstride = (half + 63) & ~(size_t)63;
    int32_t rc;
    const bool built = e->g2tab_hi == hi && e->g2tab_half == half && e->tab_owner == nullptr;
    if (!built && (rc = fold_g2_table_build(e, st, hi, half))) return rc;
    e->g2tab_hi = nullptr;
    if ((rc = jac.reserve(half * sizeof(G2J))) || (rc = e->fix_flags.reserve(4 * half + 16))) return rc;
    if (!e->sw.no_fq && half >= e->fq_min)
    {
        hipLaunchKernelGGL(HIP_KERNEL_NAME(k_fold_g2_tab_q<GlsDigits, 4>), dim3(nblk(half, 64)), dim3(64), 0, st, e->fold_tab.as<uint4>(), qstride, M, lo, (uint32_t)half, gls_wnaf(s, 4), jac.as<G2J>(), e->fix_flags.as<uint8_t>());
#if !defined(RIPP_INLINE_FALLBACK)
        hipLaunchKernelGGL(HIP_KERNEL_NAME(k_fold_g2_tab_fix<GlsDigits, 4>), dim3(FIX_GRID), dim3(64), 0, st, e->fold_tab.as<uint4>(), qstride, M, lo, (uint32_t)half, gls_wnaf(s, 4), jac.as<G2J>(), e->fix_flags.as<uint8_t>());
#endif
    }
    else
        hipLaunchKernelGGL(HIP_KERNEL_NAME(k_fold_g2_tab<GlsDigits, 4>), dim3(nblk(half, 64)), dim3(64), 0, st, e->fold_tab.as<uint4>(), qstride, M, lo, (uint32_t)half, gls_wnaf(s, 4), jac.as<G2J>());
    HIPCHK(hipGetLastError());
    return RIPP_OK;
}

int32_t job_prebuild_g2_tables(Engine* e, ripp_sipp_job* j) {
    const size_t half = j->len / 2;
    e->g2tab_hi = nullptr;
    if (e->sw.no_prebuild || e->sw.no_endo || half < 1) return RIPP_OK;
    const bool vm_form = (half <= e->vm_fold_max || half <= e->vm_joint_max) && !e->sw.no_vm;
    if (vm_form || j->pre_ready || j->pre_vm_ready || (j->tab_ready && e->tab_owner == j) || !fold_g2_table_pays(e, half)) return RIPP_OK;
    const bool xs = xscale_round(e, j, half);
    if (j->bs_on && !xs) return RIPP_OK;
    if (!fold_g2_table_fits(e, half)) return RIPP_OK;
    const G2A* b = j->b.as<G2A>();
    return fold_g2_table_build(e, e->stream, xs ? b : b + half, half);
}

int32_t job_fold(Engine* e, ripp_sipp_job* j, const Fr& x, bool allow_vm = true, bool async = false) {
    const size_t half = j->len / 2;
    int32_t rc;
    const Fr x_inv = inv(x);
    hipEvent_t t0 = e->ev_t0, t1 = e->ev_t1;
    HIPCHK(hipEventRecord(t0, e->stream));
    if (async) { hipEvent_t fa, fb; HIPCHK(hipEventCreate(&fa)); HIPCHK(hipEventCreate(&fb)); e->ev_fold_async.emplace_back(fa, fb); HIPCHK(hipEventRecord(fa, e->stream)); }
    G1A* a = j->a.as<G1A>(); G2A* b = j->b.as<G2A>();
    const size_t qstride = (half + 63) & ~(size_t)63;
    if ((rc = e->qtab.reserve(4 * G2A_CHUNKS * qstride * sizeof(uint4))) != RIPP_OK) return rc;
    const bool use_vm = allow_vm && half <= e->vm_fold_max && !e->sw.no_vm;
    const bool mid_vm = allow_vm && !use_vm && half <= e->vm_joint_max && !e->sw.no_vm && !e->sw.no_endo;
    if ((rc = e->vm_flag.reserve(sizeof(uint32_t))) != RIPP_OK) return rc;
    const bool pre = j->pre_ready && fits_128(x); j->pre_ready = false;
    const bool pre_vm = j->pre_vm_ready && fits_128(x) && allow_vm; j->pre_vm_ready = false;
    const hipStream_t g1s = e->stream2;
    HIPCHK(hipEventRecord(e->ev_fork, e->stream));
    HIPCHK(hipStreamWaitEvent(e->stream2, e->ev_fork, 0));
    const bool tab = j->tab_ready && e->tab_owner == j && fits_128(x); j->tab_ready = false;
    const int tabW = tab_width(j->tab_M);
    const G1A* tab1 = e->fold_tab1.as<G1A>() + (j->tab_fused ? half / 2 : 0);
    if (tab && !e->sw.no_fq && half >= e->fq_min)
        hipLaunchKernelGGL(k_fold_g1_tab_q, dim3(nblk(half, 256)), dim3(256), 0, g1s, tab1, j->tab_cnt, j->tab_M, a, (uint32_t)half, split32_wnaf(x, tabW), j->jac1.as<G1J>());
    else if (tab)
        hipLaunchKernelGGL(k_fold_g1_tab, dim3(nblk(half, 256)), dim3(256), 0, g1s, tab1, j->tab_cnt, j->tab_M, a, (uint32_t)half, split32_wnaf(x, tabW), j->jac1.as<G1J>());
    else if (pre)
        hipLaunchKernelGGL(k_fold_g1_two, dim3(nblk(half, 256)), dim3(256), 0, g1s, a + half, j->a_pow.as<G1A>(), a, (uint32_t)half, split64_digits(x), j->jac1.as<G1J>());
    else if (pre_vm) {
        hipLaunchKernelGGL(HIP_KERNEL_NAME(k_vm_fold_split2<Fp>), dim3(nblk(half, 4 * VM_EPW), 2), dim3(256), 4 * VM_EPW * VmCurve<Fp>::SLOTS * sizeof(VmSlot), g1s, a + half, j->a_pow_h.as<G1J>(), (uint32_t)half, split_digits_g1(x), 1, j->parts1.as<G1J>());
        hipLaunchKernelGGL(HIP_KERNEL_NAME(k_vm_combine<Fp>), dim3(nblk(half, 4 * VM_EPW)), dim3(256), 4 * VM_EPW * VmCurve<Fp>::SLOTS * sizeof(VmSlot), g1s, j->parts1.as<G1J>(), 2, a, (uint32_t)half, j->jac1.as<G1J>());
    }
    else if (use_vm || mid_vm)
        hipLaunchKernelGGL(k_vm_fold_g1, dim3(nblk(half, 4 * VM_EPW)), dim3(256), 4 * VM_EPW * VM_G1_SLOTS * sizeof(VmSlot), g1s, a + half, a, (uint32_t)half, naf_digits(x), j->jac1.as<G1J>(), e->vm_flag.as<uint32_t>());
    else if (!e->sw.no_fq && half >= e->fq_min_g1)
        hipLaunchKernelGGL(k_fold_g1_naf_q, dim3(nblk(half, 256)), dim3(256), 0, g1s, a + half, a, (uint32_t)half, naf_digits(x), j->jac1.as<G1J>());
    else
        hipLaunchKernelGGL(HIP_KERNEL_NAME(k_fold_affine_naf<Fp>), dim3(nblk(half, 256)), dim3(256), 0, g1s, a + half, a, (uint32_t)half, naf_digits(x), j->jac1.as<G1J>());
    HIPCHK(hipGetLastError());
    if ((rc = e->normalize_dev<Fp>(j->jac1.as<G1J>(), half, j->a_next.as<G1A>(), g1s)) != RIPP_OK) return rc;
    HIPCHK(hipEventRecord(e->ev_join, g1s));
    const bool xs = xscale_round(e, j, half) && fits_128(x) && (!tab || j->tab_on_lo);
    const bool unscale = j->bs_on && !xs;
    if (tab && j->tab_on_lo != xs) return (set_err("fold tables were built for the other half"), RIPP_ERR_ARG);
    const G2A* g2_hi = xs ? b : b + half; const G2A* g2_lo = xs ? b + half : b;
    const Fr g2_s = xs ? x : x_inv;
    if (unscale) {
        const Fr s_inv = inv(j->bs), sx_inv = mul(s_inv, x_inv);
        if (mid_vm) {
            GlsDigits2 d2; d2.a = gls_digits(s_inv); d2.b = gls_digits(sx_inv);
            hipLaunchKernelGGL(k_vm_fold_g2_joint2, dim3(nblk(half, 4 * VM_EPW)), dim3(256), 4 * VM_EPW * VM_G2_SLOTS * sizeof(VmSlot), e->stream, b, b + half, (uint32_t)half, d2, j->jac2.as<G2J>());
        } else {
        if ((rc = e->qtab.reserve(8 * half * sizeof(G2J))) != RIPP_OK || (rc = e->fix_flags.reserve(8 * half + 32)) != RIPP_OK) return rc;
        HIPCHK(hipStreamWaitEvent(e->stream3, e->ev_fork, 0));
        for (int t = 0; t < 2; ++t) {
            hipStream_t st2 = t ? e->stream3 : e->stream; const G2A* src = t ? b + half : b; const GlsDigits dg2 = gls_digits(t ? sx_inv : s_inv);
            G2J* parts = e->qtab.as<G2J>() + (size_t)t * 4 * half; uint8_t* flags = e->fix_flags.as<uint8_t>() + (size_t)t * ((4 * half + 15) & ~(size_t)15);
            if (!e->sw.no_fq) {
                hipLaunchKernelGGL(k_fold_g2_gls_split_q, dim3(nblk(half, 64), 4), dim3(64), 0, st2, src, (uint32_t)half, dg2, parts, flags);
#if !defined(RIPP_INLINE_FALLBACK)
                hipLaunchKernelGGL(k_fold_g2_gls_split_fix, dim3(FIX_GRID), dim3(64), 0, st2, src, (uint32_t)half, dg2, parts, flags);
#endif
            } else hipLaunchKernelGGL(k_fold_g2_gls_split, dim3(nblk(half, 64), 4), dim3(64), 0, st2, src, (uint32_t)half, dg2, parts);
        }
        HIPCHK(hipEventRecord(e->ev_join3, e->stream3)); HIPCHK(hipStreamWaitEvent(e->stream, e->ev_join3, 0));
        hipLaunchKernelGGL(k_fold_g2_combine8, dim3(nblk(half, 64)), dim3(64), 0, e->stream, e->qtab.as<G2J>(), (uint32_t)half, j->jac2.as<G2J>());
        }
        j->bs = Fr::one(); j->bs_on = false;
    } else
    if (pre_vm) {
        if (j->pre_vm_side) { HIPCHK(hipStreamWaitEvent(e->stream, e->ev_join3, 0)); j->pre_vm_side = false; }
        hipLaunchKernelGGL(HIP_KERNEL_NAME(k_vm_fold_split2<Fp2>), dim3(nblk(half, 4 * VM_EPW), 8), dim3(256), 4 * VM_EPW * VmCurve<Fp2>::SLOTS * sizeof(VmSlot), e->stream, b + half, j->b_pow_h.as<G2J>(), (uint32_t)half, split_digits_g2(x_inv), 4, j->parts2.as<G2J>());
        hipLaunchKernelGGL(HIP_KERNEL_NAME(k_vm_combine<Fp2>), dim3(nblk(half, 4 * VM_EPW)), dim3(256), 4 * VM_EPW * VmCurve<Fp2>::SLOTS * sizeof(VmSlot), e->stream, j->parts2.as<G2J>(), 8, b, (uint32_t)half, j->jac2.as<G2J>());
    } else
    if (tab && !e->sw.no_fq && half >= e->fq_min) {
        if ((rc = e->fix_flags.reserve(4 * half + 16))) return rc;
        hipLaunchKernelGGL(HIP_KERNEL_NAME(k_fold_g2_tab_q<Wnaf16, 16>), dim3(nblk(half, 64)), dim3(64), 0, e->stream, e->fold_tab.as<uint4>(), j->tab2_stride, j->tab_M, g2_lo, (uint32_t)half, gls16_wnaf(g2_s, tabW), j->jac2.as<G2J>(), e->fix_flags.as<uint8_t>());
#if !defined(RIPP_INLINE_FALLBACK)
        hipLaunchKernelGGL(HIP_KERNEL_NAME(k_fold_g2_tab_fix<Wnaf16, 16>), dim3(FIX_GRID), dim3(64), 0, e->stream, e->fold_tab.as<uint4>(), j->tab2_stride, j->tab_M, g2_lo, (uint32_t)half, gls16_wnaf(g2_s, tabW), j->jac2.as<G2J>(), e->fix_flags.as<uint8_t>());
#endif
    } else
    if (tab) {
        hipLaunchKernelGGL(HIP_KERNEL_NAME(k_fold_g2_tab<Wnaf16, 16>), dim3(nblk(half, 64)), dim3(64), 0, e->stream, e->fold_tab.as<uint4>(), j->tab2_stride, j->tab_M, g2_lo, (uint32_t)half, gls16_wnaf(g2_s, tabW), j->jac2.as<G2J>());
    } else
    if (pre) {
        if ((rc = e->qtab.reserve(8 * G2A_CHUNKS * qstride * sizeof(uint4))) != RIPP_OK) return rc;
        hipLaunchKernelGGL(k_fold_g2_gls8, dim3(nblk(half, 64)), dim3(64), 0, e->stream, b + half, j->b_pow.as<G2A>(), b, (uint32_t)half, gls8_digits(x_inv), e->qtab.as<uint4>(), qstride, j->jac2.as<G2J>());
    } else
    if (mid_vm) {
        hipLaunchKernelGGL(k_vm_fold_g2_joint, dim3(nblk(half, 4 * VM_EPW)), dim3(256), 4 * VM_EPW * VM_G2_SLOTS * sizeof(VmSlot), e->stream, g2_hi, g2_lo, (uint32_t)half, gls_digits(g2_s), j->jac2.as<G2J>());
    } else
    if (use_vm) {
        if ((rc = e->qtab.reserve(std::max<size_t>(4 * G2A_CHUNKS * qstride * sizeof(uint4), 4 * half * sizeof(G2J)))) != RIPP_OK) return rc;
        hipLaunchKernelGGL(k_vm_fold_g2_split, dim3(nblk(half, 4 * VM_EPW), 4), dim3(256), 4 * VM_EPW * VM_G2_SLOTS * sizeof(VmSlot), e->stream, b + half, (uint32_t)half, gls_digits(x_inv), e->qtab.as<G2J>(), e->vm_flag.as<uint32_t>());
        hipLaunchKernelGGL(k_vm_combine_g2, dim3(nblk(half, 4 * VM_EPW)), dim3(256), 4 * VM_EPW * VM_G2_SLOTS * sizeof(VmSlot), e->stream, e->qtab.as<G2J>(), b, (uint32_t)half, j->jac2.as<G2J>());
    } else
    if (e->sw.no_endo) {
        hipLaunchKernelGGL(HIP_KERNEL_NAME(k_fold_affine_naf<Fp2>), dim3(nblk(half, 256)), dim3(256), 0, e->stream, b + half, b, (uint32_t)half, naf_digits(x_inv), j->jac2.as<G2J>());
    } else
    if (half <= e->gls_split_max || (fold_g2_table_pays(e, half) && !(e->g2tab_hi && e->g2tab_half == half) && !fold_g2_table_fits(e, half) && ((e->mem_tier |= 16), true))) {
        if ((rc = e->qtab.reserve(std::max<size_t>(4 * G2A_CHUNKS * qstride * sizeof(uint4), 4 * half * sizeof(G2J)))) != RIPP_OK) return rc;
        if (!e->sw.no_fq) {
            if ((rc = e->fix_flags.reserve(4 * half + 16))) return rc;
            hipLaunchKernelGGL(k_fold_g2_gls_split_q, dim3(nblk(half, 64), 4), dim3(64), 0, e->stream, g2_hi, (uint32_t)half, gls_digits(g2_s), e->qtab.as<G2J>(), e->fix_flags.as<uint8_t>());
#if !defined(RIPP_INLINE_FALLBACK)
            hipLaunchKernelGGL(k_fold_g2_gls_split_fix, dim3(FIX_GRID), dim3(64), 0, e->stream, g2_hi, (uint32_t)half, gls_digits(g2_s), e->qtab.as<G2J>(), e->fix_flags.as<uint8_t>());
#endif
        }
        else hipLaunchKernelGGL(k_fold_g2_gls_split, dim3(nblk(half, 64), 4), dim3(64), 0, e->stream, g2_hi, (uint32_t)half, gls_digits(g2_s), e->qtab.as<G2J>());
        hipLaunchKernelGGL(k_fold_g2_combine, dim3(nblk(half, 64)), dim3(64), 0, e->stream, e->qtab.as<G2J>(), g2_lo, (uint32_t)half, j->jac2.as<G2J>());
    } else if (fold_g2_table_pays(e, half)) {
        if ((rc = fold_g2_table(e, e->stream, g2_hi, g2_lo, half, g2_s, j->jac2)) != RIPP_OK) return rc;
    } else {
        hipLaunchKernelGGL(k_fold_g2_gls, dim3(nblk(half, 64)), dim3(64), 0, e->stream, b + half, b, (uint32_t)half, gls_digits(x_inv), e->qtab.as<uint4>(), qstride, j->jac2.as<G2J>());
    }
    HIPCHK(hipGetLastError());
    if (xs) { j->bs = j->bs_on ? mul(j->bs, x) : x; j->bs_on = true; }
    if ((rc = e->normalize_dev<Fp2>(j->jac2.as<G2J>(), half, j->b_next.as<G2A>())) != RIPP_OK) return rc;
    HIPCHK(hipStreamWaitEvent(e->stream, e->ev_join, 0));
    HIPCHK(hipEventRecord(t1, e->stream));
    if (!async) {
        if ((rc = e->sync()) != RIPP_OK) return rc;
        float ms = 0; (void)hipEventElapsedTime(&ms, t0, t1); e->stats.fold_ms += ms;
    } else HIPCHK(hipEventRecord(e->ev_fold_async.back().second, e->stream));
    std::swap(j->a, j->a_next); std::swap(j->b, j->b_next);
    j->len = half;
    return RIPP_OK;
}

int32_t job_fold_fused(Engine* e, ripp_sipp_job* j, const Fr& x0, const Fr& x1, bool async) {
    const size_t q = j->len / 4;
    int32_t rc;
    if (!(j->tab_ready && j->tab_fused && e->tab_owner == j && j->tab_on_lo && !j->bs_on && fits_128(x0) && fits_128(x1))) { set_err("fused fold: the three-quarter tables of this job are not in place"); return RIPP_ERR_ARG; }
    j->tab_ready = false; j->pre_ready = false; j->pre_vm_ready = false;
    hipEvent_t t0 = e->ev_t0, t1 = e->ev_t1;
    HIPCHK(hipEventRecord(t0, e->stream));
    if (async) { hipEvent_t fa, fb; HIPCHK(hipEventCreate(&fa)); HIPCHK(hipEventCreate(&fb)); e->ev_fold_async.emplace_back(fa, fb); HIPCHK(hipEventRecord(fa, e->stream)); }
    if ((rc = j->jac1.reserve(q * sizeof(G1J))) || (rc = j->jac2.reserve(q * sizeof(G2J))) || (rc = e->fix_flags.reserve(2 * ((q + 15) & ~(size_t)15) + 32))) return rc;
    const int W = tab_width(j->tab_M);
    G1A* a = j->a.as<G1A>(); G2A* b = j->b.as<G2A>();
    uint8_t* flag1 = e->fix_flags.as<uint8_t>(); uint8_t* flag2 = flag1 + ((q + 15) & ~(size_t)15) + 16;
    HIPCHK(hipEventRecord(e->ev_fork, e->stream));
    HIPCHK(hipStreamWaitEvent(e->stream2, e->ev_fork, 0));
    const hipStream_t g1s = e->stream2;
    const WnafG1x4 d1 = fused_digits_g1(x0, x1, W);
    hipLaunchKernelGGL(k_fold_g1_fused_q, dim3(nblk(q, 256)), dim3(256), 0, g1s, e->fold_tab1.as<G1A>(), j->tab_cnt, j->tab_M, a, (uint32_t)q, d1, j->jac1.as<G1J>(), flag1);
    hipLaunchKernelGGL(k_fold_g1_fused_fix, dim3(FIX_GRID), dim3(64), 0, g1s, e->fold_tab1.as<G1A>(), j->tab_cnt, j->tab_M, a, (uint32_t)q, d1, j->jac1.as<G1J>(), flag1);
    HIPCHK(hipGetLastError());
    if ((rc = e->normalize_dev<Fp>(j->jac1.as<G1J>(), q, j->a_next.as<G1A>(), g1s)) != RIPP_OK) return rc;
    HIPCHK(hipEventRecord(e->ev_join, g1s));
    const Wnaf16x3 d2 = fused_digits_g2(x0, x1, W);
    hipLaunchKernelGGL(k_fold_g2_fused_q, dim3(nblk(q, 64)), dim3(64), 0, e->stream, e->fold_tab.as<uint4>(), j->tab2_stride, j->tab_M, b + 3 * q, (uint32_t)q, d2, j->jac2.as<G2J>(), flag2);
    hipLaunchKernelGGL(k_fold_g2_fused_fix, dim3(FIX_GRID), dim3(64), 0, e->stream, e->fold_tab.as<uint4>(), j->tab2_stride, j->tab_M, b + 3 * q, (uint32_t)q, d2, j->jac2.as<G2J>(), flag2);
    HIPCHK(hipGetLastError());
    j->bs = mul(x0, x1); j->bs_on = true;
    if ((rc = e->normalize_dev<Fp2>(j->jac2.as<G2J>(), q, j->b_next.as<G2A>())) != RIPP_OK) return rc;
    HIPCHK(hipStreamWaitEvent(e->stream, e->ev_join, 0));
    HIPCHK(hipEventRecord(t1, e->stream));
    if (!async) {
        if ((rc = e->sync()) != RIPP_OK) return rc;
        float ms = 0; (void)hipEventElapsedTime(&ms, t0, t1); e->stats.fold_ms += ms;
    } else HIPCHK(hipEventRecord(e->ev_fold_async.back().second, e->stream));
    std::swap(j->a, j->a_next); std::swap(j->b, j->b_next);
    j->len = q;
    return RIPP_OK;
}

void job_start_hash(ripp_sipp_job* j, const Fp12& value) {
    if (j->hash_prestarted) { j->hash_prestarted = false; return; }
    if (j->hash_thread.joinable()) j->hash_thread.join();
    j->digest_ready = false;
    const G1A* pa = j->ha_ext ? j->ha_ext : j->ha.data(); const G2A* pb = j->ha_ext ? j->hb_ext : j->hb.data(); const Fr* pr = j->ha_ext ? j->hr_ext : j->hr.data();
    const size_t pn = j->ha_ext ? j->hash_n : j->ha.size();
    j->hash_done = 0; j->hash_total = (uint64_t)pn * (96 + 192 + 32); j->hash_t0 = now_ms();
    j->hash_thread = std::thread([j, value, pa, pb, pr, pn]() { statement_digest(pa, pb, pr, pn, value, j->digest, &j->hash_done); j->digest_ready = true; });
}

}

extern "C" {

#define API __attribute__((visibility("default")))
#define LOCK std::lock_guard<std::mutex> lk_(g_mu)
#define ENGINE Engine* e; { int32_t rc_ = get_engine(&e); if (rc_ != RIPP_OK) return rc_; }

API const char* ripp_last_error(void) { return g_err.c_str(); }
static_assert(sizeof(ripp_stats) == 24 * 8, "ripp_stats changed: bump RIPP_ABI_VERSION (include/ripp_hip.h) and the bindings (ripp_amd/_lib.py, rust/ripp-hip/src/ffi.rs)");
API int32_t ripp_abi_version(void) { return RIPP_ABI_VERSION; }
API size_t ripp_stats_size(void) { return sizeof(ripp_stats); }
API void ripp_statement_hash_times(double* hash_ms, double* wait_ms) { if (hash_ms) *hash_ms = g_digest_hash_ms; if (wait_ms) *wait_ms = g_digest_wait_ms; }
API int32_t ripp_device_count(void) { int n = 0; if (hipGetDeviceCount(&n) != hipSuccess) return 0; return n; }
extern "C++" { static void vec_caches_release(); }
API int32_t ripp_init(int32_t dev) {
    LOCK;
    if (g_engine) {
        if (g_engine->device == dev) return RIPP_OK;
        if (g_live_handles.load() > 0) { set_err("ripp_init: " + std::to_string(g_live_handles.load()) + " job / SRS handle(s) are alive on device " + std::to_string(g_engine->device) + "; destroy them before re-binding the engine"); return RIPP_ERR_ARG; }
        vec_caches_release();
        g_engine->destroy(); delete g_engine; g_engine = nullptr;
    }
    Engine* e = new Engine(); int32_t rc = e->init(dev);
    if (rc != RIPP_OK) { delete e; return rc; }
    g_engine = e; return RIPP_OK;
}
API void ripp_shutdown(void) {
    LOCK; if (!g_engine) return;
    if (g_live_handles.load() > 0) { set_err("ripp_shutdown: " + std::to_string(g_live_handles.load()) + " job / SRS / vector handle(s) are still alive; destroy them first"); fprintf(stderr, "[ripp] %s\n", g_err.c_str()); return; }
    vec_caches_release();
    g_engine->destroy(); delete g_engine; g_engine = nullptr;
}
API int32_t ripp_release_scratch(void) {
    LOCK; if (!g_engine) return RIPP_OK;
    Engine* e = g_engine;
    if (hipSetDevice(e->device) != hipSuccess || hipDeviceSynchronize() != hipSuccess) { set_err("ripp_release_scratch: device synchronisation failed"); return RIPP_ERR_DEVICE; }
    for (DevBuf* b : {&e->lines, &e->partA, &e->partB, &e->jacG1, &e->jacG2, &e->tmpA, &e->tmpB, &e->tmpR, &e->affG1, &e->affG2, &e->qtab, &e->scale_tab, &e->fold_tab1, &e->fold_mult, &e->fold_tab, &e->fold_jac1, &e->fold_jac2, &e->fix_flags, &e->scale_flags}) b->release();
    e->msm_scratch[0].release(); e->msm_scratch[1].release(); e->kzg_q[0].release(); e->kzg_q[1].release(); e->kzg_bases[0].release(); e->kzg_bases[1].release();
    for (PinBuf& pb : e->stage) pb.release();
    e->tab_owner = nullptr; e->g2tab_hi = nullptr; e->job_cache.release(); vec_caches_release();
    if (e->aux) { e->aux->destroy(); delete e->aux; e->aux = nullptr; }
    for (Engine* p : e->peers) { (void)hipSetDevice(p->device); p->destroy(); delete p; }
    if (!e->peers.empty()) { e->peers.clear(); (void)hipSetDevice(e->device); }
    return RIPP_OK;
}

API size_t ripp_device_bytes(void) { return g_dev_bytes.load(std::memory_order_relaxed); }

API int32_t ripp_normalize_g1(const ripp_g1j* in, size_t n, ripp_g1a* out) {
    LOCK; ENGINE; if (n == 0) return RIPP_OK; if (!in || !out) return RIPP_ERR_ARG;
    G1J* d; int32_t rc = upload<G1J>(e, e->jacG1, in, n, &d); if (rc) return rc;
    if ((rc = e->affG1.reserve(n * sizeof(G1A)))) return rc;
    if ((rc = e->normalize_dev<Fp>(d, n, e->affG1.as<G1A>()))) return rc;
    HIPCHK(hipMemcpyAsync(out, e->affG1.p, n * sizeof(G1A), hipMemcpyDeviceToHost, e->stream));
    return e->sync();
}
API int32_t ripp_normalize_g2(const ripp_g2j* in, size_t n, ripp_g2a* out) {
    LOCK; ENGINE; if (n == 0) return RIPP_OK; if (!in || !out) return RIPP_ERR_ARG;
    G2J* d; int32_t rc = upload<G2J>(e, e->jacG2, in, n, &d); if (rc) return rc;
    if ((rc = e->affG2.reserve(n * sizeof(G2A)))) return rc;
    if ((rc = e->normalize_dev<Fp2>(d, n, e->affG2.as<G2A>()))) return rc;
    HIPCHK(hipMemcpyAsync(out, e->affG2.p, n * sizeof(G2A), hipMemcpyDeviceToHost, e->stream));
    return e->sync();
}
API int32_t ripp_scale_g1_a(const ripp_g1a* a, const ripp_fr* r, size_t n, ripp_g1a* out) {
    LOCK; ENGINE; if (n == 0) return RIPP_OK; if (!a || !r || !out) return RIPP_ERR_ARG;
    G1A* da; Fr* dr; int32_t rc;
    if ((rc = upload<G1A>(e, e->tmpA, a, n, &da))) return rc;
    if ((rc = upload<Fr>(e, e->tmpR, r, n, &dr))) return rc;
    if ((rc = e->jacG1.reserve(n * sizeof(G1J)))) return rc;
    if ((rc = e->affG1.reserve(n * sizeof(G1A)))) return rc;
    if ((rc = e->scale_g1_dev(da, 1u, dr, n, e->jacG1.as<G1J>()))) return rc;
    if ((rc = e->normalize_dev<Fp>(e->jacG1.as<G1J>(), n, e->affG1.as<G1A>()))) return rc;
    HIPCHK(hipMemcpyAsync(out, e->affG1.p, n * sizeof(G1A), hipMemcpyDeviceToHost, e->stream));
    return e->sync();
}

extern "C++" {
template <class F, bool JAC_IN, bool AFF_OUT, class IN, class OUT>
static int32_t fold_impl(const IN* hi, const IN* lo, size_t half, const ripp_fr* s, OUT* out) {
    LOCK; ENGINE; if (half == 0) return RIPP_OK; if (!hi || !lo || !s || !out) return RIPP_ERR_ARG;
    Fr sm; std::memcpy(&sm, s, sizeof(Fr));
    const ScalarBits sb = scalar_bits(sm);
    int32_t rc;
    DevBuf& jac = std::is_same<F, Fp>::value ? e->jacG1 : e->jacG2;
    DevBuf& aff = std::is_same<F, Fp>::value ? e->affG1 : e->affG2;
    if ((rc = jac.reserve(half * sizeof(Jac<F>)))) return rc;
    if (JAC_IN) {
        Jac<F>*dh, *dl;
        if ((rc = upload<Jac<F>>(e, e->tmpA, hi, half, &dh))) return rc;
        if ((rc = upload<Jac<F>>(e, e->tmpB, lo, half, &dl))) return rc;
// ... 610 lines not shown
        for (int fb = 0; fb < (1 << R); ++fb) for (int eb = 0; eb < (1 << R); ++eb) {
            int g = 0;
            for (int t = 0; t < R; ++t) g = g * 3 + (((eb >> (R - 1 - t)) & 1) - ((fb >> (R - 1 - t)) & 1) + 1);
            const size_t ia = ((size_t)eb << 1) | (side == 0 ? 1u : 0u), ib = ((size_t)fb << 1) | (side == 0 ? 0u : 1u);
            prods.push_back({a + ia * qblk, b + ib * qblk, g});
        }
        std::vector<Fp12> grows((size_t)ngroups * N_LINES); std::vector<char> gset((size_t)ngroups, 0);
        const size_t cmax = std::min<size_t>(MAX_PRODUCTS, std::max<size_t>(1, e->pairs_cap(std::min(e->max_pairs_per_batch, q * (size_t)MAX_PRODUCTS)) / q));
        const size_t nch = (prods.size() + cmax - 1) / cmax;
        auto absorb = [&](size_t c) -> int32_t {
            PinBuf& buf = j->look_rows[c & 1];
            int32_t r2 = buf.wait(); if (r2) return r2;
            const Fp12* rows = buf.as<Fp12>();
            const size_t lo = c * cmax, hi = std::min(prods.size(), lo + cmax);
            for (size_t k = lo; k < hi; ++k) {
                Fp12* dst = grows.data() + (size_t)prods[k].g * N_LINES; const Fp12* src = rows + (k - lo) * N_LINES;
                if (!gset[prods[k].g]) { std::memcpy(dst, src, N_LINES * sizeof(Fp12)); gset[prods[k].g] = 1; }
                else for (int s2 = 0; s2 < N_LINES; ++s2) dst[s2] = mul(dst[s2], src[s2]);
            }
            return RIPP_OK;
        };
        for (size_t c = 0; c < nch; ++c) {
            PinBuf& buf = j->look_rows[c & 1];
            if ((rc = buf.reserve(MAX_PRODUCTS * N_LINES * sizeof(Fp12)))) return rc;
            const size_t lo = c * cmax, hi = std::min(prods.size(), lo + cmax);
            const G1A* as[MAX_PRODUCTS]; const G2A* bs[MAX_PRODUCTS];
            for (size_t k = lo; k < hi; ++k) { as[k - lo] = prods[k].a; bs[k - lo] = prods[k].b; }
            if ((rc = e->enqueue_products(as, bs, (int)(hi - lo), 0, q, buf.as<Fp12>()))) return rc;
            HIPCHK(hipEventRecord(buf.ev, e->stream)); buf.pending = true;
            e->stats.look_pairs += (hi - lo) * q;
            if (c > 0 && (rc = absorb(c - 1))) return rc;
        }
        if ((rc = absorb(nch - 1))) return rc;
        j->look.emplace_back();
        ripp_sipp_job::LookItem& li = j->look.back();
        li.R = R; li.side = side; li.level = 0; li.npairs = q; li.q = qblk;
        for (int g = 0; g < ngroups; ++g) {
            auto rows = std::make_shared<std::vector<Fp12>>(grows.begin() + (size_t)g * N_LINES, grows.begin() + (size_t)(g + 1) * N_LINES);
            li.fe.push_back(look_pool().submit([rows]() { return final_exponentiation(miller_combine(rows->data())); }));
        }
        ++e->stats.look_items;
    }
    e->stats.look_ms += now_ms() - t0;
    if (trace_on()) fprintf(stderr, "[ripp] look-ahead: %zu of %d (round, side) values pre-evaluated in the hash window, %.1f ms (hash %s)\n", j->look.size(), items, now_ms() - t0, j->digest_ready.load() ? "already done" : "still running");
    return RIPP_OK;
}
static void look_finish_level(ripp_sipp_job::LookItem& it) {
    if (it.pend.empty()) return;
    const size_t S = it.Z.size() / 3;
    std::vector<Fp12> Zn(S);
    for (size_t r = 0; r < S; ++r) { const Fp12 lo = mul(it.pend[3 * r].get(), it.pend[3 * r + 1].get()); Zn[r] = mul(mul(lo, it.Z[S + r]), it.pend[3 * r + 2].get()); }
    it.pend.clear(); it.Z.swap(Zn); ++it.level;
}
static void look_start_level(ripp_sipp_job::LookItem& it, const GlsDigits& gx, const GlsDigits& gxi) {
    if (!it.fe.empty()) { it.Z.resize(it.fe.size()); for (size_t i = 0; i < it.fe.size(); ++i) it.Z[i] = it.fe[i].get(); it.fe.clear(); }
    const size_t S = it.Z.size() / 3;
    for (size_t r = 0; r < S; ++r) {
        const Fp12 zm = it.Z[r], zp = it.Z[2 * S + r];
        it.pend.push_back(host_pool().submit([zm, gxi]() { return gt_pow_gls_strings(zm, gxi, 3u); }));
        it.pend.push_back(host_pool().submit([zm, gxi]() { return gt_pow_gls_strings(zm, gxi, 12u); }));
        it.pend.push_back(host_pool().submit([zp, gx]() { return gt_pow_gls_strings(zp, gx, 15u); }));
    }
}
static void look_apply(ripp_sipp_job* j, size_t t, const Fr& x) {
    bool any = false; for (auto& it : j->look) any = any || (size_t)it.R > t;
    if (!any) return;
    const GlsDigits gx = gls_digits(x), gxi = gls_digits(inv(x));
    for (int pass = 0; pass < 2; ++pass) for (auto& it : j->look) {
        if ((size_t)it.R <= t || ((size_t)it.R == t + 1) != (pass == 0)) continue;
        look_finish_level(it);
        look_start_level(it, gx, gxi);
    }
}
static ripp_sipp_job::LookItem* look_find(ripp_sipp_job* j, size_t round, int side) { for (auto& it : j->look) if ((size_t)it.R == round && it.side == side) return &it; return nullptr; }
static bool look_full(ripp_sipp_job* j, size_t round) { const auto* l = look_find(j, round, 0); const auto* r = look_find(j, round, 1); return l && r && l->npairs == l->q && r->npairs == r->q; }

static int32_t job_round0_shared(Engine* e, ripp_sipp_job* j, Fp12* rows) {
    const size_t q = j->len / 4;
    const G1A* a = j->a.as<G1A>(); const G2A* b = j->b.as<G2A>();
    const G1A* as[8] = {a + 2 * q, a + q, a + 3 * q,   a, a + q, a + 3 * q,   a + 3 * q,   a + q};
    const G2A* bs[8] = {b, b, b,   b + 2 * q, b + 2 * q, b + 2 * q,   b + q,   b + 3 * q};
    std::vector<Fp12> all((size_t)8 * N_LINES);
    const double t0 = now_ms();
    int32_t rc = e->step_products(as, bs, 8, q, all.data());
    e->stats.miller_products_ms += now_ms() - t0;
    if (rc) return rc;
    auto row = [&](int p) { return all.data() + (size_t)p * N_LINES; };
    for (int s2 = 0; s2 < N_LINES; ++s2) { rows[s2] = mul(row(0)[s2], row(6)[s2]); rows[N_LINES + s2] = mul(row(3)[s2], row(7)[s2]); }
    j->look.clear();
    j->look.emplace_back();
    ripp_sipp_job::LookItem& li = j->look.back();
    li.R = 1; li.side = 0; li.level = 0; li.npairs = q; li.q = q;
    for (int g = 0; g < 3; ++g) {
        auto grows = std::make_shared<std::vector<Fp12>>((size_t)N_LINES);
        for (int s2 = 0; s2 < N_LINES; ++s2) (*grows)[s2] = g == 0 ? row(4)[s2] : g == 1 ? mul(row(1)[s2], row(5)[s2]) : row(2)[s2];
        li.fe.push_back(look_pool().submit([grows]() { return final_exponentiation(miller_combine(grows->data())); }));
    }
    ++e->stats.look_items; e->stats.look_pairs += 4 * q;
    return RIPP_OK;
}

static std::atomic<int> g_fail_rank{-1}, g_fail_round{-1};
static bool test_fail_hit(int rank, size_t round) {
    if (g_fail_rank.load(std::memory_order_relaxed) == rank && g_fail_round.load(std::memory_order_relaxed) == 1000 + (int)round) raise(SIGKILL);
    if (g_fail_rank.load(std::memory_order_relaxed) != rank || g_fail_round.load(std::memory_order_relaxed) != (int)round) return false;
    g_fail_rank = -1; g_fail_round = -1;
    set_err("injected failure (ripp_test_inject_failure) in the fold of round " + std::to_string(round) + " on rank " + std::to_string(rank));
    return true;
}
struct SippPlanMsg { uint64_t n_local; int32_t world, rank, look_items, window, rc, pad; double hash_left_ms; };
struct SippRoundMsg { Fp12 z[2]; uint8_t digest[32]; int32_t rc, pad[3]; };
struct SippTailMsg { G1A a; G2A b; int32_t rc, pad[3]; };
static int32_t sipp_prove_core(Engine* e, ripp_sipp_job* j, const Fp12& val, const uint8_t* seed_digest, ripp_gt* proof, ripp_fr* challenges, ripp_stats* st) {
    const int world0 = j->world0, rank = j->rank;
    const double t_start = now_ms();
    double exchange_ms = 0;
    comm_mark_proof();
    e->mem_tier = 0;
    struct Quiesce { Engine* e; ripp_sipp_job* j; ~Quiesce() {
        (void)hipStreamSynchronize(e->stream); (void)hipStreamSynchronize(e->stream2); (void)hipStreamSynchronize(e->stream3);
        j->tp_round[0] = j->tp_round[1] = ~(size_t)0; j->pre_vm_ready = false; j->pre_vm_side = false; j->pre_ready = false; j->tab_ready = false; j->look.clear();
        e->g2tab_hi = nullptr;
        if (j->hash_thread.joinable()) j->hash_thread.join();
        j->ha_ext = nullptr; j->hb_ext = nullptr; j->hr_ext = nullptr; j->hash_prestarted = false; } } quiesce{e, j};
    const bool window = rank == 0 && !seed_digest;
    if (rank == 0) {
        if (seed_digest) { if (j->hash_thread.joinable()) j->hash_thread.join(); std::memcpy(j->digest, seed_digest, 32); j->digest_ready = true; j->hash_prestarted = false; }
        else job_start_hash(j, val);
    }
    const bool look_forced = e->look_eighths >= 0;
    int look_items = (rank == 0 || look_forced) ? look_plan(e, j->n_local, world0, window || look_forced) : 0;
    j->no_window = !window; j->look_deadline = 0;
    if (world0 > 1) {
        double hash_left = 0;
        if (window && j->hash_total > 0) hash_left = std::max(0.0, (double)j->hash_total / (e->cal_hash_bytes_per_ms > 0 ? e->cal_hash_bytes_per_ms : 1.17e6) - (now_ms() - j->hash_t0));
        SippPlanMsg mine{(uint64_t)j->n_local, world0, rank, look_items, window ? 1 : 0, RIPP_OK, 0, hash_left};
        std::vector<SippPlanMsg> all((size_t)world0);
        const double tx = now_ms();
        t_ex_kind = EX_PLAN;
        int32_t rc = comm_allgather(e, &mine, all.data(), sizeof mine); if (rc) return rc;
        exchange_ms += now_ms() - tx;
        for (int w = 0; w < world0; ++w) {
            if (all[w].rc) { set_err("sharded SIPP proof: rank " + std::to_string(w) + " failed before the proof started (status " + std::to_string(all[w].rc) + ")"); return RIPP_ERR_DEVICE; }
            if (all[w].n_local != (uint64_t)j->n_local || all[w].world != world0 || all[w].rank != w) { set_err("sharded SIPP proof: the ranks disagree on the shard size / world size / rank order"); return RIPP_ERR_ARG; }
        }
        look_items = all[0].look_items; j->no_window = !all[0].window;
        if (rank != 0 && all[0].window && all[0].hash_left_ms > 0) j->look_deadline = now_ms() + all[0].hash_left_ms;
    }
    struct HotOff { ~HotOff() { host_pool().set_hot(false); } } hot_off;
    struct QuietOff { Engine* e; ~QuietOff() { e->quiet_waits = false; } } quiet_off{e};
    e->quiet_waits = window && e->quiet_waits_cfg;
    j->look_rows[0].blocking = j->look_rows[1].blocking = e->quiet_waits;
    struct XsOff { ripp_sipp_job* j; ~XsOff() { j->xs_enabled = false; } } xs_off{j};
    j->xs_enabled = true; j->seeded = false;
    int32_t lrc = job_begin(e, j);
    if (lrc && world0 == 1) return lrc;
    e->stats.look_items = 0; e->stats.look_pairs = 0; e->stats.look_ms = 0;
    if (trace_on()) fprintf(stderr, "[ripp] scale+normalize done at t=%.1f ms\n", now_ms() - t_start);
    size_t len = j->n_local;
    bool sharded = world0 > 1, digest_sent = world0 == 1;
    size_t round = 0;
    Fr x_prev = Fr::zero();
    bool fuse_pending = false; Fr x0_saved = Fr::zero();
    j->tp_round[0] = j->tp_round[1] = ~(size_t)0;
    while ((sharded ? len * (size_t)world0 : len) > 1) {
        if (sharded && len == 1) {
            SippTailMsg mine; std::memset((void*)&mine, 0, sizeof mine);
            if (!lrc) {
                auto grab = [&]() -> int32_t {
                    HIPCHK(hipStreamSynchronize(e->stream2)); HIPCHK(hipStreamSynchronize(e->stream3));
                    HIPCHK(hipMemcpyAsync(&mine.a, j->a.p, sizeof(G1A), hipMemcpyDeviceToHost, e->stream));
                    HIPCHK(hipMemcpyAsync(&mine.b, j->b.p, sizeof(G2A), hipMemcpyDeviceToHost, e->stream));
                    return e->sync(); };
                lrc = grab();
            }
            mine.rc = lrc;
            std::vector<SippTailMsg> all((size_t)world0);
            const double tx = now_ms();
            int32_t rc = comm_allgather(e, &mine, all.data(), sizeof mine); if (rc) return rc;
            exchange_ms += now_ms() - tx;
            for (int w = 0; w < world0; ++w) if (all[w].rc) { if (!lrc) set_err("sharded SIPP proof: rank " + std::to_string(w) + " failed (status " + std::to_string(all[w].rc) + ")"); return lrc ? lrc : RIPP_ERR_DEVICE; }
            const size_t L = (size_t)world0;
            if ((rc = j->a.reserve(L * sizeof(G1A))) || (rc = j->b.reserve(L * sizeof(G2A))) || (rc = j->a_next.reserve(L * sizeof(G1A))) ||
                (rc = j->b_next.reserve(L * sizeof(G2A))) || (rc = j->jac1.reserve(L * sizeof(G1J))) || (rc = j->jac2.reserve(L * sizeof(G2J))) || (rc = e->stage[3].reserve(L * (sizeof(G1A) + sizeof(G2A))))) return rc;
            G1A* ha = e->stage[3].as<G1A>(); G2A* hb = reinterpret_cast<G2A*>(ha + L);
            for (size_t w = 0; w < L; ++w) { ha[w] = all[w].a; hb[w] = all[w].b; }
            if (j->bs_on) { set_err("sharded SIPP proof: the G2 vector is still x-scaled at the tail gather"); return RIPP_ERR_ARG; }
            HIPCHK(hipMemcpyAsync(j->a.p, ha, L * sizeof(G1A), hipMemcpyHostToDevice, e->stream));
            HIPCHK(hipMemcpyAsync(j->b.p, hb, L * sizeof(G2A), hipMemcpyHostToDevice, e->stream));
            if ((rc = e->sync())) return rc;
            j->len = len = L; j->world = 1; sharded = false;
            j->pre_vm_ready = false;
            continue;
        }
        Fp12 rows[2 * N_LINES];
        const double tr0 = now_ms();
        ripp_sipp_job::LookItem* lk_l = lrc ? nullptr : look_find(j, round, 0);
        ripp_sipp_job::LookItem* lk_r = lrc ? nullptr : look_find(j, round, 1);
        const bool tp_round = !lrc && j->tp_round[round & 1] == round;
        double t0 = tr0;
        double round0_ms_per_pair = 7.7e-5;
        bool shared_r0 = false;
        Fp12 zl = Fp12::one(), zr = Fp12::one();
        auto local_values = [&]() -> int32_t {
            int32_t rc;
            const size_t half = fuse_pending ? j->len / 4 : j->len / 2;
            const size_t start[2] = {lk_l ? std::min(lk_l->npairs, half) : 0, lk_r ? std::min(lk_r->npairs, half) : 0};
            const bool dev[2] = {!tp_round && start[0] < half, !tp_round && start[1] < half};
            if (dev[0] && dev[1] && start[0] == 0 && start[1] == 0) {
                const double tp = now_ms();
                shared_r0 = round == 0 && !j->seeded && look_items >= 8 && j->len >= 4 && !e->sw.no_share && !e->sw.no_precompute && (look_forced || !j->digest_ready.load());
                if (shared_r0) { if ((rc = job_round0_shared(e, j, rows))) return rc; }
                else if ((rc = job_round_partials(e, j, rows))) return rc;
                if (round == 0 && j->len >= ((size_t)1 << 16)) {
                    round0_ms_per_pair = (now_ms() - tp) / (double)(shared_r0 ? 2 * j->len : j->len);
                    if (e->ranks_per_device <= 1.0) e->cal_ms_per_pair = round0_ms_per_pair;
                }
            }
            else for (int sd = 0; sd < 2; ++sd) {
                if (!dev[sd]) continue;
                const G1A* as[1] = {j->a.as<G1A>() + (sd == 0 ? half : 0) + start[sd]}; const G2A* bs[1] = {j->b.as<G2A>() + (sd == 0 ? 0 : half) + start[sd]};
                const double tp = now_ms();
                if ((rc = e->step_products(as, bs, 1, half - start[sd], rows + sd * N_LINES))) return rc;
                e->stats.miller_products_ms += now_ms() - tp;
            }
            if (round >= 1 && !fuse_pending && !tp_round && (rc = job_prebuild_g2_tables(e, j))) return rc;
            const bool plan_fuse = look_forced ? look_items >= 16 : look_items >= 12;
            if (round == 0 && !j->seeded && (rc = job_precompute_round0(e, j, (plan_fuse || e->sw.fuse_tables) && j->len >= 4))) return rc;
            if (!j->pre_vm_ready && (rc = job_precompute_vm(e, j))) return rc;
            const bool next_known = round == 0 ? (plan_fuse && j->len >= 4 && (look_forced || !j->digest_ready.load())) : look_full(j, round + 1);
            if (!tp_round && !next_known && tail_pipe_ok(e, j) && (rc = job_tail_enqueue(e, j, round + 1))) return rc;
            t0 = now_ms();
            if (tp_round) { if ((rc = job_tail_values(j, round, x_prev, &zl, &zr))) return rc; }
            else {
                Fp12 zd[2] = {Fp12::one(), Fp12::one()};
                if (dev[0] && dev[1]) pairing_values(rows, 2, zd);
                else if (dev[0]) pairing_values(rows, 1, &zd[0]);
                else if (dev[1]) pairing_values(rows + N_LINES, 1, &zd[1]);
                if (j->bs_on && (dev[0] || dev[1])) {
                    const GlsDigits gsi = gls_digits(inv(j->bs));
                    if (host_pool().size() >= 11) {
                        Fp12 part[8];
                        host_pool().parallel(8, [&](int t) { if (!dev[t >> 2]) return; part[t] = gt_pow_gls_strings(zd[t >> 2], gsi, 1u << (t & 3)); });
                        for (int k = 0; k < 2; ++k) if (dev[k]) zd[k] = mul(mul(part[4 * k], part[4 * k + 1]), mul(part[4 * k + 2], part[4 * k + 3]));
                    } else {
                    Fp12 part[4];
                    host_pool().parallel(4, [&](int t) { if (!dev[t >> 1]) return; part[t] = gt_pow_gls_strings(zd[t >> 1], gsi, (t & 1) ? 12u : 3u); });
                    for (int k = 0; k < 2; ++k) if (dev[k]) zd[k] = mul(part[2 * k], part[2 * k + 1]);
                    }
                }
                zl = zd[0]; zr = zd[1];
                if (lk_l) { look_finish_level(*lk_l); zl = dev[0] ? mul(lk_l->Z[0], zd[0]) : lk_l->Z[0]; }
                if (lk_r) { look_finish_level(*lk_r); zr = dev[1] ? mul(lk_r->Z[0], zd[1]) : lk_r->Z[0]; }
            }
            if (round == 0 && !j->seeded && (rc = job_lookahead(e, j, look_items, look_forced, round0_ms_per_pair, shared_r0 ? 1 : 0))) return rc;
            return RIPP_OK;
        };
        if (!lrc) lrc = local_values();
        if (lrc && !sharded) return lrc;
        if (!j->seeded && rank == 0) {
            const double th = now_ms();
            if (j->hash_thread.joinable()) j->hash_thread.join();
            e->stats.hash_ms += now_ms() - th;
        }
        if (sharded || !digest_sent) {
            SippRoundMsg mine; std::memset((void*)&mine, 0, sizeof mine);
            mine.z[0] = zl; mine.z[1] = zr; mine.rc = lrc;
            if (rank == 0) std::memcpy(mine.digest, j->digest, 32);
            std::vector<SippRoundMsg> all((size_t)world0);
            const double tx = now_ms();
            int32_t rc = comm_allgather(e, &mine, all.data(), sizeof mine); if (rc) return rc;
            exchange_ms += now_ms() - tx;
            for (int w = 0; w < world0; ++w) if (all[w].rc) { if (!lrc) set_err("sharded SIPP proof: rank " + std::to_string(w) + " failed (status " + std::to_string(all[w].rc) + ")"); return lrc ? lrc : RIPP_ERR_DEVICE; }
            if (sharded) { zl = all[0].z[0]; zr = all[0].z[1]; for (int w = 1; w < world0; ++w) { zl = mul(zl, all[w].z[0]); zr = mul(zr, all[w].z[1]); } }
            if (!digest_sent) { std::memcpy(j->digest, all[0].digest, 32); digest_sent = true; }
        }
        if (!j->seeded) {
            j->rng.from_digest(j->digest); j->seeded = true;
            e->quiet_waits = false;
            host_pool().set_hot(e->hot_workers_cfg ? (e->hot_workers_cfg == 1 && effective_cpus() >= (int)host_pool().size() + 2) : hot_workers_pay(world0));
        }
        const Fr x = fs::sipp_challenge(j->rng, zl, zr);
        x_prev = x;
        look_apply(j, round, x);
        e->stats.host_ms += now_ms() - t0;
        std::memcpy(&proof[2 * round], &zl, sizeof(Fp12)); std::memcpy(&proof[2 * round + 1], &zr, sizeof(Fp12));
        if (challenges) std::memcpy(&challenges[round], &x, sizeof(Fr));
        const double tf0 = now_ms();
        const bool pipelined = j->tp_round[(round + 1) & 1] == round + 1;
        const bool known = look_full(j, round + 1);
        if (!sharded && len == 2) { j->len = 0; j->pre_vm_ready = false; }
        else {
            if (!lrc && test_fail_hit(rank, round)) lrc = RIPP_ERR_DEVICE;
            if (!lrc && fuse_pending) { lrc = job_fold_fused(e, j, x0_saved, x, pipelined || known); fuse_pending = false; }
            else if (!lrc && round == 0 && known && j->tab_ready && j->tab_fused && e->tab_owner == j && !j->bs_on) { fuse_pending = true; x0_saved = x; }
            else
            if (!lrc) lrc = job_fold(e, j, x, true, pipelined || known);
            if (!lrc && pipelined) {
                if (!j->pre_vm_ready) lrc = job_precompute_vm(e, j, true);
                if (!lrc && tail_pipe_ok(e, j)) lrc = job_tail_enqueue(e, j, round + 2);
            }
            if (lrc && !sharded) return lrc;
        }
        len /= 2;
        if (trace_on()) fprintf(stderr, "[ripp] round %2zu len %8zu: products %.2f ms, host %.2f ms, fold %.2f ms%s (t=%.1f)\n", round, len * 2, t0 - tr0, tf0 - t0, now_ms() - tf0, (pipelined || known) ? " (enqueued)" : "", now_ms() - t_start);
        ++round;
    }
    if (j->hash_thread.joinable()) j->hash_thread.join();
    host_pool().set_hot(false);
    if (lrc) return lrc;
    int32_t rc;
    if ((rc = e->sync())) return rc; HIPCHK(hipStreamSynchronize(e->stream2)); HIPCHK(hipStreamSynchronize(e->stream3));
    e->collect_kernel_stats();
    e->stats.exchange_ms = exchange_ms;
    e->stats.mem_tier = (uint64_t)e->mem_tier; e->stats.device_bytes = g_dev_bytes.load();
    e->stats.statement_hash_ms = window ? g_digest_hash_ms : 0; e->stats.statement_hash_wait_ms = window ? g_digest_wait_ms : 0;
    if (window && j->hash_total >= ((uint64_t)336 << 16) && g_digest_hash_ms + g_digest_wait_ms > 1.0) e->cal_hash_bytes_per_ms = (double)j->hash_total / (g_digest_hash_ms + g_digest_wait_ms);
    e->stats.total_ms = now_ms() - t_start;
    if (st) *st = e->stats;
    return RIPP_OK;
}

static void config_from_engine(const Engine* e, ripp_config* c) {
    std::memset(c, 0, sizeof *c); c->struct_size = (uint32_t)sizeof *c;
    c->no_vm = e->sw.no_vm; c->no_precompute = e->sw.no_precompute; c->no_fold_tables = e->sw.no_fold_tables; c->no_msm_glv = e->sw.no_msm_glv; c->lp_one_lane = e->sw.lp_one_lane;
    c->no_endo = e->sw.no_endo; c->no_fq = e->sw.no_fq; c->no_xscale = e->sw.no_xscale; c->no_share = e->sw.no_share; c->no_fuse = e->sw.no_fuse; c->fuse_tables = e->sw.fuse_tables; c->scale_no_fq = e->scale_no_fq; c->agg_sequential = e->agg_sequential; c->look_static = e->look_static; c->quiet_waits = e->quiet_waits_cfg;
    c->look_eighths = e->look_eighths; c->ranks_per_device = (int32_t)e->ranks_per_device; c->msm_c = e->msm_tune.c; c->msm_ch = e->msm_tune.ch; c->msm_gmin = e->msm_tune.gmin; c->no_prebuild = e->sw.no_prebuild;
    c->vm_lines_max = e->vm_lines_max; c->vm_fold_max = e->vm_fold_max; c->vm_tree_max = e->vm_tree_max; c->gls_split_max = e->gls_split_max; c->msm_vm_merge_max = e->msm_vm_merge_max; c->fold_tab_min = e->fold_tab_min;
    c->fq_min = e->fq_min; c->lp_fq_min = e->lp_fq_min; c->vm_joint_max = e->vm_joint_max; c->vm_scale_max = e->vm_scale_max; c->tail_pipe_max = e->tail_pipe_max; c->ml_fq_min = e->ml_fq_min; c->fq_min_g1 = e->fq_min_g1; c->msm_lds_sort_min = e->msm_lds_sort_min; c->msm_chunk_min = e->msm_chunk_min;
    c->mem_cap_bytes = e->mem_cap; c->hot_workers = (uint32_t)e->hot_workers_cfg; c->no_job_cache = e->sw.no_job_cache;
    c->no_lp_karatsuba = e->sw.no_lp_kara; c->comm_timeout_ms = e->comm_timeout_ms; c->plan_derate_pct = e->plan_derate_pct; c->n_devices = e->n_devices_cfg;
}
API int32_t ripp_config_default(ripp_config* cfg) {
    if (!cfg) return RIPP_ERR_ARG;
    Engine tmp; tmp.defaults = Engine::Sizes{tmp.vm_lines_max, tmp.vm_fold_max, tmp.vm_tree_max, tmp.gls_split_max, tmp.msm_vm_merge_max, tmp.fold_tab_min, tmp.fq_min, tmp.lp_fq_min, tmp.vm_joint_max, tmp.vm_scale_max, tmp.tail_pipe_max, tmp.ml_fq_min, tmp.fq_min_g1, tmp.msm_lds_sort_min, tmp.msm_chunk_min};
    config_from_engine(&tmp, cfg); cfg->look_eighths = -1; cfg->ranks_per_device = 1;
    return RIPP_OK;
}
API int32_t ripp_configure(const ripp_config* cfg) {
    LOCK;
    if (!cfg) { g_cfg_set = false; return RIPP_OK; }
    if (cfg->struct_size != sizeof(ripp_config)) { set_err("ripp_configure: struct_size does not match this library's ripp_config (fill the struct with ripp_config_default first)"); return RIPP_ERR_ARG; }
    g_cfg = *cfg; g_cfg_set = true;
    return RIPP_OK;
}
API int32_t ripp_config_get(ripp_config* cfg) {
    if (!cfg) return RIPP_ERR_ARG;
    LOCK; ENGINE;
    config_from_engine(e, cfg);
    return RIPP_OK;
}

API void ripp_test_inject_failure(int32_t rank, int32_t round) { g_fail_rank = rank; g_fail_round = round; }

API int32_t ripp_sipp_job_prove(ripp_sipp_job* j, const ripp_gt* value, ripp_gt* proof, ripp_fr* challenges, ripp_stats* st) {
    LOCK; ENGINE; if (!j || !value || !proof || j->world0 != 1) return RIPP_ERR_ARG;
    Fp12 val; std::memcpy(&val, value, sizeof(Fp12));
    return sipp_prove_core(e, j, val, nullptr, proof, challenges, st);
}

extern "C++" {
// ... 134 lines not shown
```

### ripp_amd/csrc/fq_curve2.hpp

```cpp
#pragma once
#include "fq_curve.hpp"

namespace ripp {

#if defined(__HIP_DEVICE_COMPILE__)
#if defined(RIPP_BLS12_377)
constexpr int FQ2_BETA = 5;
#else
constexpr int FQ2_BETA = 1;
#endif
template <uint64_t L1, int V1> __device__ __forceinline__ auto fq_mul_beta(const Fq<L1, V1>& a) {
    if constexpr (FQ2_BETA == 1) return a;
    else { static_assert(FQ2_BETA == 5, "FQ2_BETA"); return fq_add(fq_dbl(fq_dbl(a)), a); }
}
template <uint64_t LM = FQ_LN, int VB = 2> struct Fq2T { Fq<LM, VB> c0, c1; };
using Fq2n = Fq2T<FQ_LN, 2>;
using Fq2C = Fq2T<FQ_LN, 4>;

template <uint64_t L1, int V1, uint64_t L2, int V2> __device__ __forceinline__ auto f2_add(const Fq2T<L1, V1>& a, const Fq2T<L2, V2>& b) { return Fq2T<L1 + L2 - 1, V1 + V2>{fq_add(a.c0, b.c0), fq_add(a.c1, b.c1)}; }
template <uint64_t L1, int V1, uint64_t L2, int V2> __device__ __forceinline__ auto f2_sub(const Fq2T<L1, V1>& a, const Fq2T<L2, V2>& b) { return Fq2T<fq28::sub_lm(L1, L2), V1 + V2 + 1>{fq_sub(a.c0, b.c0), fq_sub(a.c1, b.c1)}; }
template <uint64_t L1, int V1> __device__ __forceinline__ auto f2_dbl(const Fq2T<L1, V1>& a) { return Fq2T<2 * L1 - 1, 2 * V1>{fq_dbl(a.c0), fq_dbl(a.c1)}; }
template <uint64_t L1, int V1> __device__ __forceinline__ auto f2_norm(const Fq2T<L1, V1>& a) { return Fq2T<FQ_LN, V1>{fq_norm(a.c0), fq_norm(a.c1)}; }
template <uint64_t L1, int V1> __device__ __forceinline__ Fq2n f2_reduce(const Fq2T<L1, V1>& a) { return {fq_reduce(a.c0), fq_reduce(a.c1)}; }
template <uint64_t L1, int V1> __device__ __forceinline__ Fq2C f2_coord(const Fq2T<L1, V1>& a) { return {fq_coord(a.c0), fq_coord(a.c1)}; }
// ... 171 lines not shown
    if (!linf) bad |= jmadd2_q(acc, [&]() { return f2_from(opaque(lp)->x); }, [&]() { return f2_from(opaque(lp)->y); }, park);
#if !defined(RIPP_INLINE_FALLBACK)
    flag[i] = bad;
    if (!bad) out[i] = G2J{f2_to(acc.x), f2_to(acc.y), f2_to(acc.z)};
#else
    if (bad) fold_g2_tab_complete<D, NS>(qtab, stride, M, lo, i, dg, out);
    else out[i] = G2J{f2_to(acc.x), f2_to(acc.y), f2_to(acc.z)};
#endif
#endif
}
template <class D, int NS>
__global__ void __launch_bounds__(64) k_fold_g2_tab_fix(const uint4* __restrict__ qtab, size_t stride, int M, const G2A* __restrict__ lo, uint32_t half, D dg, G2J* __restrict__ out, const uint8_t* __restrict__ flag) {
    for_flagged(flag, half, [&](uint32_t i) { fold_g2_tab_complete<D, NS>(qtab, stride, M, lo, i, dg, out); });
}

struct Wnaf16x3 { Wnaf16 s[3]; int len; };
__device__ __noinline__ inline void fold_g2_fused_complete(const uint4* __restrict__ qtab, size_t stride, int M, const G2A* __restrict__ lo, uint32_t q, uint32_t i, const Wnaf16x3& dg, G2J* __restrict__ out) {
    G2J acc = jac_inf<Fp2>();
#pragma unroll 1
    for (int pos = dg.len - 1; pos >= 0; --pos) {
        acc = dbl(acc);
#pragma unroll 1
        for (int u = 0; u < 3; ++u) {
#pragma unroll 1
            for (int t = 0; t < 16; ++t) {
                const int d = dg.s[u].d[t][pos];
                if (d != 0) {
                    G2A p = load_chunks<G2A_CHUNKS, G2A>(qtab, (size_t)t * M + ((d < 0 ? -d : d) >> 1), stride, (size_t)u * q + i);
                    if (d < 0) p.y = neg(p.y);
                    acc = add_mixed(acc, p);
                }
            }
        }
    }
    out[i] = add_mixed(acc, lo[i]);
}
__global__ void __launch_bounds__(64, 2) k_fold_g2_fused_q(const uint4* __restrict__ qtab, size_t stride, int M, const G2A* __restrict__ lo, uint32_t q, Wnaf16x3 dg, G2J* __restrict__ out, uint8_t* __restrict__ flag) {
    __shared__ uint4 park_[7 * 64];
    const uint32_t i = blockIdx.x * blockDim.x + threadIdx.x;
    if (i >= q) return;
#if defined(__HIP_DEVICE_COMPILE__)
    uint4* park = park_ + threadIdx.x;
    JacQ2 acc; j2_set_identity(acc);
    bool inf = true, bad = false;
#pragma unroll 1
    for (int pos = dg.len - 1; pos >= 0; --pos) {
        if (!inf) jdbl2_q(acc);
#pragma unroll 1
        for (int ut = 0; ut < 48; ++ut) {
            const int u = ut >> 4, t = ut & 15;
            const int d = dg.s[u].d[t][pos];
            if (d == 0) continue;
            uint32_t il = i; asm volatile("" : "+v"(il));
            const uint4* base = qtab + ((size_t)t * M + ((d < 0 ? -d : d) >> 1)) * G2A_CHUNKS * stride + (size_t)u * q + il;
            auto ldfp2 = [&](int q0) { Fp2 v; uint4* dd = reinterpret_cast<uint4*>(&v); const uint4* b2 = opaque(base);
#pragma unroll
                for (int c = 0; c < 6; ++c) dd[c] = b2[(size_t)(q0 + c) * stride]; return v; };
#if defined(RIPP_BLS12_377)
            auto loadx = [&]() { return f2_from(ldfp2(0)); };
            auto loady = [&]() { const Fp2 y = ldfp2(6); return f2_from(d < 0 ? neg(y) : y); };
#else
            auto loadx = [&]() { return f2_tab(ldfp2(0)); };
            auto loady = [&]() { return f2_tab_y(ldfp2(6), d < 0); };
#endif
            if (inf) {
                const Fp2 x0 = ldfp2(0), y0 = ldfp2(6);
                bad |= x0.is_zero() && y0.is_zero();
                j2_set(acc, f2_from(x0), f2_from(d < 0 ? neg(y0) : y0), Fq2n{fq_one(), fq_zero()}); inf = false;
            } else {
                { const Fp2 x0 = ldfp2(0); bad |= x0.is_zero() && ldfp2(6).is_zero(); }
                bad |= jmadd2_q(acc, loadx, loady, park);
            }
        }
    }
    const G2A* lp = lo + i;
    if (inf) { out[i] = to_jac(*lp); flag[i] = 0; return; }
    bool linf; { const G2A l = *lp; linf = is_inf(l); }
    if (!linf) bad |= jmadd2_q(acc, [&]() { return f2_from(opaque(lp)->x); }, [&]() { return f2_from(opaque(lp)->y); }, park);
    flag[i] = bad;
    if (!bad) out[i] = G2J{f2_to(acc.x), f2_to(acc.y), f2_to(acc.z)};
#endif
}
__global__ void __launch_bounds__(64) k_fold_g2_fused_fix(const uint4* __restrict__ qtab, size_t stride, int M, const G2A* __restrict__ lo, uint32_t q, Wnaf16x3 dg, G2J* __restrict__ out, const uint8_t* __restrict__ flag) {
    for_flagged(flag, q, [&](uint32_t i) { fold_g2_fused_complete(qtab, stride, M, lo, q, i, dg, out); });
}

template <class F>
__device__ __noinline__ void odd_multiples_complete(const Affine<F>* __restrict__ base, uint32_t n, int M, uint32_t i, Jac<F>* __restrict__ out) {
    const Affine<F> b = base[i];
    const Jac<F> b2 = dbl(to_jac(b));
    Jac<F> t = add_mixed(b2, b);
    out[i] = t;
#pragma unroll 1
    for (int m = 1; m < M - 1; ++m) { t = add(t, b2); out[(size_t)m * n + i] = t; }
}
__global__ void __launch_bounds__(64, 2) k_odd_multiples_q(const G2A* __restrict__ base, uint32_t n, int M, G2J* __restrict__ out, uint8_t* __restrict__ flag) {
    __shared__ uint4 park_[14 * 64];
    const uint32_t i = blockIdx.x * blockDim.x + threadIdx.x;
    if (i >= n || M < 2) return;
#if defined(__HIP_DEVICE_COMPILE__)
    uint4* park = park_ + threadIdx.x;
    uint4* zpark = park + 7 * 64;
    auto st7 = [](uint4* dst, size_t stride, const Fq2n& v) { uint32_t w[28];
#pragma unroll
        for (int k = 0; k < 14; ++k) { w[k] = v.c0.l[k]; w[14 + k] = v.c1.l[k]; }
        const uint4* src = reinterpret_cast<const uint4*>(w);
#pragma unroll
        for (int k = 0; k < 7; ++k) dst[k * stride] = src[k]; };
    auto ld7 = [](const uint4* src, size_t stride) { uint4 q[7];
#pragma unroll
        for (int k = 0; k < 7; ++k) q[k] = src[k * stride];
        const uint32_t* w = reinterpret_cast<const uint32_t*>(q);
        Fq2n v;
#pragma unroll
        for (int k = 0; k < 14; ++k) { v.c0.l[k] = w[k]; v.c1.l[k] = w[14 + k]; }
        return v; };
    const G2A* bp = base + i;
    bool bad;
    { const G2A b = *bp; bad = is_inf(b); }
    uint4* tmp = reinterpret_cast<uint4*>(out + (size_t)(M - 2) * n + i);
    JacQ2 t;
    {
        JacQ2 d; j2_set(d, f2_from(opaque(bp)->x), f2_from(opaque(bp)->y), Fq2n{fq_one(), fq_zero()});
        f2_pin(d.z);
        jdbl2_q(d);
        Fq2n Z2 = f2_reduce(d.z); f2_pin(Z2);
        bad |= f2_is_zero(Z2);
        st7(zpark, 64, Z2);
        st7(tmp, 1, f2_reduce(d.x)); st7(tmp + 7, 1, f2_reduce(d.y));
        Fq2n zz = f2_sqrd(Z2); f2_pin(zz);
        { Fq2n px = f2_muld(f2_from(opaque(bp)->x), zz); f2_pin(px); t.x = f2_slot<Fq2X>(px); }
        Fq2n zzz = f2_muld(zz, Z2); f2_pin(zzz);
        { Fq2n py = f2_muld(f2_from(opaque(bp)->y), zzz); f2_pin(py); t.y = f2_slot<Fq2Y>(py); }
        t.z = f2_slot<Fq2Z>(Fq2n{fq_one(), fq_zero()}); f2_pin(t.z);
    }
#pragma unroll 1
    for (int m = 0; m < M - 1; ++m) {
        bad |= jmadd2_q(t, [&]() { return ld7(opaque(tmp), 1); }, [&]() { return ld7(opaque(tmp) + 7, 1); }, park);
        Fq2n zo = f2_muld(t.z, ld7(zpark, 64)); f2_pin(zo);
        out[(size_t)m * n + i] = G2J{f2_to(t.x), f2_to(t.y), f2_to(zo)};
    }
#if !defined(RIPP_INLINE_FALLBACK)
    flag[i] = bad;
#else
    if (bad) odd_multiples_complete<Fp2>(base, n, M, i, out);
#endif
#endif
}
__global__ void __launch_bounds__(64) k_odd_multiples_fix(const G2A* __restrict__ base, uint32_t n, int M, G2J* __restrict__ out, const uint8_t* __restrict__ flag) {
    if (M < 2) return;
    for_flagged(flag, n, [&](uint32_t i) { odd_multiples_complete<Fp2>(base, n, M, i, out); });
}

__device__ __noinline__ inline G2J fold_g2_gls_split_complete(const G2A& q, const GlsDigits& dg, int j) {
    G2J acc = jac_inf<Fp2>();
#pragma unroll 1
    for (int pos = dg.len - 1; pos >= 0; --pos) {
        acc = dbl(acc);
        const int d = dg.d[j][pos];
        if (d != 0) { G2A t = q; if (d < 0) t.y = neg(t.y); acc = add_mixed(acc, t); }
    }
    return acc;
}
__global__ void __launch_bounds__(64, 2) k_fold_g2_gls_split_q(const G2A* __restrict__ hi, uint32_t half, GlsDigits dg, G2J* __restrict__ parts , uint8_t* __restrict__ flag ) {
    __shared__ uint4 park_[21 * 64];
    const uint32_t i = blockIdx.x * blockDim.x + threadIdx.x;
    if (i >= half) return;
    const int j = blockIdx.y;
#if defined(__HIP_DEVICE_COMPILE__)
    uint4* park = park_ + threadIdx.x;
    uint4* qpark = park + 7 * 64;
    auto st7 = [](uint4* dst, const Fq2n& v) { uint32_t w[28];
#pragma unroll
        for (int k = 0; k < 14; ++k) { w[k] = v.c0.l[k]; w[14 + k] = v.c1.l[k]; }
        const uint4* src = reinterpret_cast<const uint4*>(w);
#pragma unroll
        for (int k = 0; k < 7; ++k) dst[k * 64] = src[k]; };
    auto ld7 = [](const uint4* src) { uint4 q[7];
#pragma unroll
        for (int k = 0; k < 7; ++k) q[k] = src[k * 64];
        const uint32_t* w = reinterpret_cast<const uint32_t*>(q);
        Fq2n v;
#pragma unroll
        for (int k = 0; k < 14; ++k) { v.c0.l[k] = w[k]; v.c1.l[k] = w[14 + k]; }
        return v; };
    bool bad;
    {
        const G2A q = gls_image(hi[i], j);
        bad = is_inf(q);
        st7(qpark, f2_from(q.x)); st7(qpark + 7 * 64, f2_from(q.y));
    }
    JacQ2 acc; j2_set_identity(acc);
    bool inf = true;
#pragma unroll 1
    for (int pos = dg.len - 1; pos >= 0; --pos) {
        if (!inf) jdbl2_q(acc);
        const int d = dg.d[j][pos];
        if (d == 0) continue;
        auto loadx = [&]() { return ld7(qpark); };
        auto loady = [&]() { const Fq2n y = ld7(qpark + 7 * 64); if (d > 0) return y; return Fq2n{fq_reduce(fq_neg(y.c0)), fq_reduce(fq_neg(y.c1))}; };
        if (inf) { j2_set(acc, loadx(), loady(), Fq2n{fq_one(), fq_zero()}); f2_pin(acc.z); inf = false; }
        else bad |= jmadd2_q(acc, loadx, loady, park);
    }
#if !defined(RIPP_INLINE_FALLBACK)
    flag[(size_t)j * half + i] = bad;
    if (bad) return;
#else
    if (bad) { parts[(size_t)j * half + i] = fold_g2_gls_split_complete(gls_image(hi[i], j), dg, j); return; }
#endif
    if (inf) parts[(size_t)j * half + i] = jac_inf<Fp2>();
    else parts[(size_t)j * half + i] = G2J{f2_to(acc.x), f2_to(acc.y), f2_to(acc.z)};
#endif
}
__global__ void __launch_bounds__(64) k_fold_g2_gls_split_fix(const G2A* __restrict__ hi, uint32_t half, GlsDigits dg, G2J* __restrict__ parts, const uint8_t* __restrict__ flag) {
    for_flagged(flag, 4 * half, [&](uint32_t f) { const int j = (int)(f / half); const uint32_t i = f - (uint32_t)j * half; parts[f] = fold_g2_gls_split_complete(gls_image(hi[i], j), dg, j); });
}

__global__ void __launch_bounds__(64, 2) k_pow2_mul_g2_q(const G2A* __restrict__ in, uint32_t n, int k, G2J* __restrict__ out) {
    const uint32_t i = blockIdx.x * blockDim.x + threadIdx.x;
    if (i >= n) return;
#if defined(__HIP_DEVICE_COMPILE__)
    const G2A* bp = in + i;
    bool inf; { const G2A b = *bp; inf = is_inf(b); }
    if (inf) { out[i] = jac_inf<Fp2>(); return; }
    JacQ2 d; j2_set(d, f2_from(opaque(bp)->x), f2_from(opaque(bp)->y), Fq2n{fq_one(), fq_zero()});
    f2_pin(d.z);
#pragma unroll 1
    for (int t = 0; t < k; ++t) jdbl2_q(d);
    out[i] = G2J{f2_to(d.x), f2_to(d.y), f2_to(d.z)};
#endif
}

}
```

Before: 2.652 million.

## Precompute 2^16-power G2 bases on side stream to shorten GLS split fold chains

Adds a precompute step that runs on a side stream. It computes 2^16, 2^32 and 2^48 multiples of the high-half G2 bases ahead of the next fold round. The fold then splits each GLS base-u digit into four 16-bit chunks, giving 16 parallel short NAF chains of about 18 doublings instead of 4 chains of about 66, and combines them per element. This moves doubling work off the critical path and raises parallelism. The cost is extra memory (3 affine + 16 Jacobian parts per element), extra combine adds, and a normalize pass on the side stream. It only applies to mid-size rounds with half up to 2^16.

After: 2.635 million (median of 2 runs). No clear change (-0.6%).

```diff
diff --git a/ripp_amd/csrc/engine.hip b/ripp_amd/csrc/engine.hip
--- a/ripp_amd/csrc/engine.hip
+++ b/ripp_amd/csrc/engine.hip
@@ -212,6 +212,7 @@
     int device = -1;
     hipStream_t stream = nullptr, stream2 = nullptr;
     hipEvent_t ev_fork = nullptr, ev_join = nullptr, ev_join3 = nullptr;
+    hipEvent_t ev_sb_fork = nullptr, ev_sb = nullptr;
     hipEvent_t ev_t0 = nullptr, ev_t1 = nullptr;
     int n_simd = 1024;
     DevBuf lines, partA, partB, jacG1, jacG2, tmpA, tmpB, tmpR, affG1, affG2;
@@ -246,6 +247,8 @@
     std::vector<std::pair<hipEvent_t, hipEvent_t>> ev_fold_async;
     size_t tail_pipe_max = (size_t)1 << 11;
     size_t vm_tree_max = (size_t)1 << 16;
+    size_t sb_fold_max = (size_t)1 << 16;
+    static constexpr size_t SB_FOLD_CAP = (size_t)1 << 16;
     size_t vm_fold_max = (size_t)1 << 11;
     DevBuf vm_flag;
     size_t vm_lines_max = (size_t)1 << 15;
@@ -309,6 +312,7 @@
         env_sz("RIPP_GLS_SPLIT_MAX", gls_split_max); env_sz("RIPP_MSM_VM_MERGE_MAX", msm_vm_merge_max); env_sz("RIPP_FOLD_TAB_MIN", fold_tab_min);
         env_sz("RIPP_FQ_MIN", fq_min); env_sz("RIPP_LP_FQ_MIN", lp_fq_min); env_sz("RIPP_VM_JOINT_MAX", vm_joint_max);
         env_sz("RIPP_MSM_LDS_SORT_MIN", msm_lds_sort_min); env_sz("RIPP_MSM_CHUNK_MIN", msm_chunk_min);
+        sb_fold_max = (size_t)1 << 16; env_sz("RIPP_SB_FOLD_MAX", sb_fold_max);
         env_sz("RIPP_VM_SCALE_MAX", vm_scale_max); env_sz("RIPP_TAIL_PIPE_MAX", tail_pipe_max); env_sz("RIPP_ML_FQ_MIN", ml_fq_min); env_sz("RIPP_FQ_MIN_G1", fq_min_g1);
         auto env_on = [](const char* k, bool& v) { if (std::getenv(k)) v = true; };
         env_on("RIPP_NO_VM", sw.no_vm); env_on("RIPP_NO_PRECOMPUTE", sw.no_precompute); env_on("RIPP_NO_FOLD_TABLES", sw.no_fold_tables); env_on("RIPP_NO_MSM_GLV", sw.no_msm_glv);
@@ -347,6 +351,7 @@
         HIPCHK(hipStreamCreateWithFlags(&stream4, hipStreamNonBlocking)); HIPCHK(hipEventCreateWithFlags(&ev_join4, hipEventDisableTiming));
         HIPCHK(hipStreamCreateWithFlags(&stream5, hipStreamNonBlocking)); HIPCHK(hipEventCreateWithFlags(&ev_join5, hipEventDisableTiming));
         HIPCHK(hipEventCreateWithFlags(&ev_fork, hipEventDisableTiming)); HIPCHK(hipEventCreateWithFlags(&ev_join, hipEventDisableTiming)); HIPCHK(hipEventCreateWithFlags(&ev_join3, hipEventDisableTiming));
+        HIPCHK(hipEventCreateWithFlags(&ev_sb_fork, hipEventDisableTiming)); HIPCHK(hipEventCreateWithFlags(&ev_sb, hipEventDisableTiming));
         HIPCHK(hipEventCreate(&ev_t0)); HIPCHK(hipEventCreate(&ev_t1));
         { hipDeviceProp_t pr; if (hipGetDeviceProperties(&pr, dev) == hipSuccess) n_simd = pr.multiProcessorCount * 4; }
         defaults = Sizes{vm_lines_max, vm_fold_max, vm_tree_max, gls_split_max, msm_vm_merge_max, fold_tab_min, fq_min, lp_fq_min, vm_joint_max, vm_scale_max, tail_pipe_max, ml_fq_min, fq_min_g1, msm_lds_sort_min, msm_chunk_min};
@@ -371,6 +376,7 @@
         if (stream) (void)hipStreamDestroy(stream);
         if (stream2) (void)hipStreamDestroy(stream2);
         if (ev_fork) (void)hipEventDestroy(ev_fork); if (ev_join) (void)hipEventDestroy(ev_join); if (ev_join3) (void)hipEventDestroy(ev_join3);
+        if (ev_sb_fork) (void)hipEventDestroy(ev_sb_fork); if (ev_sb) (void)hipEventDestroy(ev_sb);
         if (ev_t0) (void)hipEventDestroy(ev_t0); if (ev_t1) (void)hipEventDestroy(ev_t1);
         if (ev_quiet) (void)hipEventDestroy(ev_quiet);
     }
@@ -697,23 +703,41 @@
     nd.len = naf_recode(c.l, 8, nd.d, 258);
     return nd;
 }
-GlsDigits gls_digits(const Fr& s_mont) {
+void gls_base_u(const Fr& s_mont, uint64_t d[4]) {
     const Fr c = from_mont(s_mont);
     uint64_t v[4] = {(uint64_t)c.l[0] | ((uint64_t)c.l[1] << 32), (uint64_t)c.l[2] | ((uint64_t)c.l[3] << 32),
                      (uint64_t)c.l[4] | ((uint64_t)c.l[5] << 32), (uint64_t)c.l[6] | ((uint64_t)c.l[7] << 32)};
+    for (int j = 0; j < 4; ++j) {
+        unsigned __int128 rem = 0;
+        for (int i = 3; i >= 0; --i) { const unsigned __int128 cur = (rem << 64) | v[i]; v[i] = (uint64_t)(cur / BLS_X_ABS); rem = cur % BLS_X_ABS; }
+        d[j] = (uint64_t)rem;
+    }
+}
+GlsDigits gls_digits(const Fr& s_mont) {
+    uint64_t d[4]; gls_base_u(s_mont, d);
     GlsDigits g; std::memset(&g, 0, sizeof g);
     int maxlen = 0;
     for (int j = 0; j < 4; ++j) {
-        unsigned __int128 rem = 0;
-        for (int i = 3; i >= 0; --i) { const unsigned __int128 cur = (rem << 64) | v[i]; v[i] = (uint64_t)(cur / BLS_X_ABS); rem = cur % BLS_X_ABS; }
-        const uint64_t dj = (uint64_t)rem;
-        const uint32_t words[2] = {(uint32_t)dj, (uint32_t)(dj >> 32)};
+        const uint32_t words[2] = {(uint32_t)d[j], (uint32_t)(d[j] >> 32)};
         const int len = naf_recode(words, 2, g.d[j], 66);
         if (len > maxlen) maxlen = len;
     }
     g.len = maxlen;
     return g;
 }
+#if !defined(RIPP_BLS12_377)
+SbDigits sb_digits(const Fr& s_mont) {
+    uint64_t d[4]; gls_base_u(s_mont, d);
+    SbDigits g; std::memset(&g, 0, sizeof g);
+    for (int j = 0; j < 4; ++j) for (int b = 0; b < 4; ++b) {
+        const uint32_t words[1] = {(uint32_t)((d[j] >> (16 * b)) & 0xFFFFu)};
+        const int len = naf_recode(words, 1, g.d[4 * b + j], 18);
+        if (len > 0) g.mask |= 1u << (4 * b + j);
+        if (len > g.len) g.len = len;
+    }
+    return g;
+}
+#endif
 
 void glv_split(const Fr& s_mont, uint32_t rem[9], uint32_t quo[8]) {
     const Fr c = from_mont(s_mont);
@@ -915,6 +939,7 @@
     std::atomic<uint64_t> hash_done{0}; uint64_t hash_total = 0; double hash_t0 = 0;
     bool no_window = false;
     size_t hash_n = 0;
+    bool sb_ready = false; const G2A* sb_hi = nullptr; size_t sb_half = 0;
     DevBuf a_pow_h, b_pow_h, parts1, parts2; bool pre_vm_ready = false, pre_vm_side = false;
     PinBuf tp_rows[2]; size_t tp_round[2] = {~(size_t)0, ~(size_t)0};
     std::vector<G1A> ha; std::vector<G2A> hb; std::vector<Fr> hr;
@@ -1120,12 +1145,36 @@
     e->g2tab_hi = nullptr;
     if (e->sw.no_prebuild || e->sw.no_endo || half < 1) return RIPP_OK;
     const bool vm_form = (half <= e->vm_fold_max || half <= e->vm_joint_max) && !e->sw.no_vm;
-    if (vm_form || j->pre_ready || j->pre_vm_ready || (j->tab_ready && e->tab_owner == j) || !fold_g2_table_pays(e, half)) return RIPP_OK;
+    if (vm_form || j->sb_ready || j->pre_ready || j->pre_vm_ready || (j->tab_ready && e->tab_owner == j) || !fold_g2_table_pays(e, half)) return RIPP_OK;
     const bool xs = xscale_round(e, j, half);
     if (j->bs_on && !xs) return RIPP_OK;
     if (!fold_g2_table_fits(e, half)) return RIPP_OK;
     const G2A* b = j->b.as<G2A>();
     return fold_g2_table_build(e, e->stream, xs ? b : b + half, half);
+}
+
+int32_t job_precompute_sb(Engine* e, ripp_sipp_job* j) {
+    j->sb_ready = false;
+#if !defined(RIPP_BLS12_377)
+    const size_t half = j->len / 2;
+    if (half <= e->vm_fold_max || half > std::min(e->sb_fold_max, Engine::SB_FOLD_CAP) || e->sw.no_precompute || e->sw.no_endo || e->sw.no_fq) return RIPP_OK;
+    if (j->pre_ready || j->pre_vm_ready || (j->tab_ready && e->tab_owner == j)) return RIPP_OK;
+    const bool xs = xscale_round(e, j, half);
+    if (j->bs_on && !xs) return RIPP_OK;
+    const size_t need = 3 * half * sizeof(G2A) + 16 * half * sizeof(G2J);
+    if (!e->mem_fits(need, j->b_pow.cap + j->parts2.cap)) return RIPP_OK;
+    int32_t rc;
+    if ((rc = j->b_pow.reserve(3 * half * sizeof(G2A))) || (rc = j->parts2.reserve(16 * half * sizeof(G2J))) || (rc = e->fix_flags.reserve(16 * half + 16))) return rc;
+    const G2A* hi = xs ? j->b.as<G2A>() : j->b.as<G2A>() + half;
+    HIPCHK(hipEventRecord(e->ev_sb_fork, e->stream));
+    HIPCHK(hipStreamWaitEvent(e->stream3, e->ev_sb_fork, 0));
+    hipLaunchKernelGGL(k_pow2_steps_g2_q, dim3(nblk(half, 64)), dim3(64), 0, e->stream3, hi, (uint32_t)half, 16, 3, j->parts2.as<G2J>());
+    HIPCHK(hipGetLastError());
+    if ((rc = e->normalize_dev<Fp2>(j->parts2.as<G2J>(), 3 * half, j->b_pow.as<G2A>(), e->stream3))) return rc;
+    HIPCHK(hipEventRecord(e->ev_sb, e->stream3));
+    j->sb_hi = hi; j->sb_half = half; j->sb_ready = true;
+#endif
+    return RIPP_OK;
 }
 
 int32_t job_fold(Engine* e, ripp_sipp_job* j, const Fr& x, bool allow_vm = true, bool async = false) {
@@ -1173,7 +1222,12 @@
     if (tab && j->tab_on_lo != xs) return (set_err("fold tables were built for the other half"), RIPP_ERR_ARG);
     const G2A* g2_hi = xs ? b : b + half; const G2A* g2_lo = xs ? b + half : b;
     const Fr g2_s = xs ? x : x_inv;
+    const bool sb_done = j->sb_ready; j->sb_ready = false;
+    if (sb_done) HIPCHK(hipStreamWaitEvent(e->stream, e->ev_sb, 0));
+    const bool sb = sb_done && j->sb_half == half && j->sb_hi == g2_hi && !unscale && !pre_vm && !tab && !pre && !e->sw.no_fq;
+    const char* g2_form = "";
     if (unscale) {
+        g2_form = mid_vm ? "joint2" : "gls_split x2";
         const Fr s_inv = inv(j->bs), sx_inv = mul(s_inv, x_inv);
         if (mid_vm) {
             GlsDigits2 d2; d2.a = gls_digits(s_inv); d2.b = gls_digits(sx_inv);
@@ -1196,12 +1250,23 @@
         }
         j->bs = Fr::one(); j->bs_on = false;
     } else
+#if !defined(RIPP_BLS12_377)
+    if (sb) {
+        g2_form = "sb_split";
+        const SbDigits dg = sb_digits(g2_s);
+        hipLaunchKernelGGL(k_fold_g2_sb_split_q, dim3(nblk(half, 64), 16), dim3(64), 0, e->stream, g2_hi, j->b_pow.as<G2A>(), (uint32_t)half, dg, j->parts2.as<G2J>(), e->fix_flags.as<uint8_t>());
+        hipLaunchKernelGGL(k_fold_g2_sb_split_fix, dim3(FIX_GRID), dim3(64), 0, e->stream, g2_hi, j->b_pow.as<G2A>(), (uint32_t)half, dg, j->parts2.as<G2J>(), e->fix_flags.as<uint8_t>());
+        hipLaunchKernelGGL(k_fold_g2_sb_combine, dim3(nblk(half, 64)), dim3(64), 0, e->stream, j->parts2.as<G2J>(), dg.mask, g2_lo, (uint32_t)half, j->jac2.as<G2J>());
+    } else
+#endif
     if (pre_vm) {
+        g2_form = "vm_split2";
         if (j->pre_vm_side) { HIPCHK(hipStreamWaitEvent(e->stream, e->ev_join3, 0)); j->pre_vm_side = false; }
         hipLaunchKernelGGL(HIP_KERNEL_NAME(k_vm_fold_split2<Fp2>), dim3(nblk(half, 4 * VM_EPW), 8), dim3(256), 4 * VM_EPW * VmCurve<Fp2>::SLOTS * sizeof(VmSlot), e->stream, b + half, j->b_pow_h.as<G2J>(), (uint32_t)half, split_digits_g2(x_inv), 4, j->parts2.as<G2J>());
         hipLaunchKernelGGL(HIP_KERNEL_NAME(k_vm_combine<Fp2>), dim3(nblk(half, 4 * VM_EPW)), dim3(256), 4 * VM_EPW * VmCurve<Fp2>::SLOTS * sizeof(VmSlot), e->stream, j->parts2.as<G2J>(), 8, b, (uint32_t)half, j->jac2.as<G2J>());
     } else
     if (tab && !e->sw.no_fq && half >= e->fq_min) {
+        g2_form = "round0_tab_q";
         if ((rc = e->fix_flags.reserve(4 * half + 16))) return rc;
         hipLaunchKernelGGL(HIP_KERNEL_NAME(k_fold_g2_tab_q<Wnaf16, 16>), dim3(nblk(half, 64)), dim3(64), 0, e->stream, e->fold_tab.as<uint4>(), j->tab2_stride, j->tab_M, g2_lo, (uint32_t)half, gls16_wnaf(g2_s, tabW), j->jac2.as<G2J>(), e->fix_flags.as<uint8_t>());
 #if !defined(RIPP_INLINE_FALLBACK)
@@ -1209,24 +1274,30 @@
 #endif
     } else
     if (tab) {
+        g2_form = "round0_tab";
         hipLaunchKernelGGL(HIP_KERNEL_NAME(k_fold_g2_tab<Wnaf16, 16>), dim3(nblk(half, 64)), dim3(64), 0, e->stream, e->fold_tab.as<uint4>(), j->tab2_stride, j->tab_M, g2_lo, (uint32_t)half, gls16_wnaf(g2_s, tabW), j->jac2.as<G2J>());
     } else
     if (pre) {
+        g2_form = "gls8";
         if ((rc = e->qtab.reserve(8 * G2A_CHUNKS * qstride * sizeof(uint4))) != RIPP_OK) return rc;
         hipLaunchKernelGGL(k_fold_g2_gls8, dim3(nblk(half, 64)), dim3(64), 0, e->stream, b + half, j->b_pow.as<G2A>(), b, (uint32_t)half, gls8_digits(x_inv), e->qtab.as<uint4>(), qstride, j->jac2.as<G2J>());
     } else
     if (mid_vm) {
+        g2_form = "joint";
         hipLaunchKernelGGL(k_vm_fold_g2_joint, dim3(nblk(half, 4 * VM_EPW)), dim3(256), 4 * VM_EPW * VM_G2_SLOTS * sizeof(VmSlot), e->stream, g2_hi, g2_lo, (uint32_t)half, gls_digits(g2_s), j->jac2.as<G2J>());
     } else
     if (use_vm) {
+        g2_form = "vm_split";
         if ((rc = e->qtab.reserve(std::max<size_t>(4 * G2A_CHUNKS * qstride * sizeof(uint4), 4 * half * sizeof(G2J)))) != RIPP_OK) return rc;
         hipLaunchKernelGGL(k_vm_fold_g2_split, dim3(nblk(half, 4 * VM_EPW), 4), dim3(256), 4 * VM_EPW * VM_G2_SLOTS * sizeof(VmSlot), e->stream, b + half, (uint32_t)half, gls_digits(x_inv), e->qtab.as<G2J>(), e->vm_flag.as<uint32_t>());
         hipLaunchKernelGGL(k_vm_combine_g2, dim3(nblk(half, 4 * VM_EPW)), dim3(256), 4 * VM_EPW * VM_G2_SLOTS * sizeof(VmSlot), e->stream, e->qtab.as<G2J>(), b, (uint32_t)half, j->jac2.as<G2J>());
     } else
     if (e->sw.no_endo) {
+        g2_form = "naf";
         hipLaunchKernelGGL(HIP_KERNEL_NAME(k_fold_affine_naf<Fp2>), dim3(nblk(half, 256)), dim3(256), 0, e->stream, b + half, b, (uint32_t)half, naf_digits(x_inv), j->jac2.as<G2J>());
     } else
     if (half <= e->gls_split_max || (fold_g2_table_pays(e, half) && !(e->g2tab_hi && e->g2tab_half == half) && !fold_g2_table_fits(e, half) && ((e->mem_tier |= 16), true))) {
+        g2_form = "gls_split";
         if ((rc = e->qtab.reserve(std::max<size_t>(4 * G2A_CHUNKS * qstride * sizeof(uint4), 4 * half * sizeof(G2J)))) != RIPP_OK) return rc;
         if (!e->sw.no_fq) {
             if ((rc = e->fix_flags.reserve(4 * half + 16))) return rc;
@@ -1238,11 +1309,14 @@
         else hipLaunchKernelGGL(k_fold_g2_gls_split, dim3(nblk(half, 64), 4), dim3(64), 0, e->stream, g2_hi, (uint32_t)half, gls_digits(g2_s), e->qtab.as<G2J>());
         hipLaunchKernelGGL(k_fold_g2_combine, dim3(nblk(half, 64)), dim3(64), 0, e->stream, e->qtab.as<G2J>(), g2_lo, (uint32_t)half, j->jac2.as<G2J>());
     } else if (fold_g2_table_pays(e, half)) {
+        g2_form = "tab";
         if ((rc = fold_g2_table(e, e->stream, g2_hi, g2_lo, half, g2_s, j->jac2)) != RIPP_OK) return rc;
     } else {
+        g2_form = "gls";
         hipLaunchKernelGGL(k_fold_g2_gls, dim3(nblk(half, 64)), dim3(64), 0, e->stream, b + half, b, (uint32_t)half, gls_digits(x_inv), e->qtab.as<uint4>(), qstride, j->jac2.as<G2J>());
     }
     HIPCHK(hipGetLastError());
+    if (trace_on()) fprintf(stderr, "[ripp] fold to %zu: G2 form %s%s%s\n", half, g2_form, xs ? " (x-scaled)" : "", sb_done && !sb ? ", second bases unused" : "");
     if (xs) { j->bs = j->bs_on ? mul(j->bs, x) : x; j->bs_on = true; }
     if ((rc = e->normalize_dev<Fp2>(j->jac2.as<G2J>(), half, j->b_next.as<G2A>())) != RIPP_OK) return rc;
     HIPCHK(hipStreamWaitEvent(e->stream, e->ev_join, 0));
@@ -2159,7 +2233,7 @@
     e->quiet_waits = window && e->quiet_waits_cfg;
     j->look_rows[0].blocking = j->look_rows[1].blocking = e->quiet_waits;
     struct XsOff { ripp_sipp_job* j; ~XsOff() { j->xs_enabled = false; } } xs_off{j};
-    j->xs_enabled = true; j->seeded = false;
+    j->xs_enabled = true; j->seeded = false; j->sb_ready = false;
     int32_t lrc = job_begin(e, j);
     if (lrc && world0 == 1) return lrc;
     e->stats.look_items = 0; e->stats.look_pairs = 0; e->stats.look_ms = 0;
@@ -2214,6 +2288,7 @@
             const size_t half = fuse_pending ? j->len / 4 : j->len / 2;
             const size_t start[2] = {lk_l ? std::min(lk_l->npairs, half) : 0, lk_r ? std::min(lk_r->npairs, half) : 0};
             const bool dev[2] = {!tp_round && start[0] < half, !tp_round && start[1] < half};
+            if (round >= 1 && !fuse_pending && !tp_round && j->seeded && (rc = job_precompute_sb(e, j))) return rc;
             if (dev[0] && dev[1] && start[0] == 0 && start[1] == 0) {
                 const double tp = now_ms();
                 shared_r0 = round == 0 && !j->seeded && look_items >= 8 && j->len >= 4 && !e->sw.no_share && !e->sw.no_precompute && (look_forced || !j->digest_ready.load());
diff --git a/ripp_amd/csrc/fq_curve2.hpp b/ripp_amd/csrc/fq_curve2.hpp
--- a/ripp_amd/csrc/fq_curve2.hpp
+++ b/ripp_amd/csrc/fq_curve2.hpp
@@ -347,21 +347,17 @@
     for_flagged(flag, n, [&](uint32_t i) { odd_multiples_complete<Fp2>(base, n, M, i, out); });
 }
 
-__device__ __noinline__ inline G2J fold_g2_gls_split_complete(const G2A& q, const GlsDigits& dg, int j) {
+__device__ __noinline__ inline G2J fold_g2_gls_split_complete(const G2A& q, const int8_t* __restrict__ dj, int len) {
     G2J acc = jac_inf<Fp2>();
 #pragma unroll 1
-    for (int pos = dg.len - 1; pos >= 0; --pos) {
+    for (int pos = len - 1; pos >= 0; --pos) {
         acc = dbl(acc);
-        const int d = dg.d[j][pos];
+        const int d = dj[pos];
         if (d != 0) { G2A t = q; if (d < 0) t.y = neg(t.y); acc = add_mixed(acc, t); }
     }
     return acc;
 }
-__global__ void __launch_bounds__(64, 2) k_fold_g2_gls_split_q(const G2A* __restrict__ hi, uint32_t half, GlsDigits dg, G2J* __restrict__ parts , uint8_t* __restrict__ flag ) {
-    __shared__ uint4 park_[21 * 64];
-    const uint32_t i = blockIdx.x * blockDim.x + threadIdx.x;
-    if (i >= half) return;
-    const int j = blockIdx.y;
+__device__ __forceinline__ bool fold_g2_split_lane_q(const G2A* __restrict__ src, int j, const int8_t* __restrict__ dj, int len, G2J* __restrict__ part, uint4* park_) {
 #if defined(__HIP_DEVICE_COMPILE__)
     uint4* park = park_ + threadIdx.x;
     uint4* qpark = park + 7 * 64;
@@ -381,34 +377,83 @@
         return v; };
     bool bad;
     {
-        const G2A q = gls_image(hi[i], j);
+        const G2A q = gls_image(*src, j);
         bad = is_inf(q);
         st7(qpark, f2_from(q.x)); st7(qpark + 7 * 64, f2_from(q.y));
     }
     JacQ2 acc; j2_set_identity(acc);
     bool inf = true;
 #pragma unroll 1
-    for (int pos = dg.len - 1; pos >= 0; --pos) {
+    for (int pos = len - 1; pos >= 0; --pos) {
         if (!inf) jdbl2_q(acc);
-        const int d = dg.d[j][pos];
+        const int d = dj[pos];
         if (d == 0) continue;
         auto loadx = [&]() { return ld7(qpark); };
         auto loady = [&]() { const Fq2n y = ld7(qpark + 7 * 64); if (d > 0) return y; return Fq2n{fq_reduce(fq_neg(y.c0)), fq_reduce(fq_neg(y.c1))}; };
         if (inf) { j2_set(acc, loadx(), loady(), Fq2n{fq_one(), fq_zero()}); f2_pin(acc.z); inf = false; }
         else bad |= jmadd2_q(acc, loadx, loady, park);
     }
+    if (bad) return true;
+    if (inf) *part = jac_inf<Fp2>();
+    else *part = G2J{f2_to(acc.x), f2_to(acc.y), f2_to(acc.z)};
+#endif
+    return false;
+}
+__global__ void __launch_bounds__(64, 2) k_fold_g2_gls_split_q(const G2A* __restrict__ hi, uint32_t half, GlsDigits dg, G2J* __restrict__ parts , uint8_t* __restrict__ flag ) {
+    __shared__ uint4 park_[21 * 64];
+    const uint32_t i = blockIdx.x * blockDim.x + threadIdx.x;
+    if (i >= half) return;
+    const int j = blockIdx.y;
+    const size_t f = (size_t)j * half + i;
+    const bool bad = fold_g2_split_lane_q(hi + i, j, dg.d[j], dg.len, parts + f, park_);
 #if !defined(RIPP_INLINE_FALLBACK)
-    flag[(size_t)j * half + i] = bad;
-    if (bad) return;
-#else
-    if (bad) { parts[(size_t)j * half + i] = fold_g2_gls_split_complete(gls_image(hi[i], j), dg, j); return; }
-#endif
-    if (inf) parts[(size_t)j * half + i] = jac_inf<Fp2>();
-    else parts[(size_t)j * half + i] = G2J{f2_to(acc.x), f2_to(acc.y), f2_to(acc.z)};
+    flag[f] = bad;
+#else
+    if (bad) parts[f] = fold_g2_gls_split_complete(gls_image(hi[i], j), dg.d[j], dg.len);
 #endif
 }
 __global__ void __launch_bounds__(64) k_fold_g2_gls_split_fix(const G2A* __restrict__ hi, uint32_t half, GlsDigits dg, G2J* __restrict__ parts, const uint8_t* __restrict__ flag) {
-    for_flagged(flag, 4 * half, [&](uint32_t f) { const int j = (int)(f / half); const uint32_t i = f - (uint32_t)j * half; parts[f] = fold_g2_gls_split_complete(gls_image(hi[i], j), dg, j); });
+    for_flagged(flag, 4 * half, [&](uint32_t f) { const int j = (int)(f / half); const uint32_t i = f - (uint32_t)j * half; parts[f] = fold_g2_gls_split_complete(gls_image(hi[i], j), dg.d[j], dg.len); });
+}
+
+struct SbDigits { int8_t d[16][20]; int len; uint32_t mask; };
+__device__ __forceinline__ const G2A* fold_g2_sb_src(const G2A* __restrict__ hi, const G2A* __restrict__ pow, uint32_t half, int t, uint32_t i) { const int b = t >> 2; return b == 0 ? hi + i : pow + (size_t)(b - 1) * half + i; }
+__global__ void __launch_bounds__(64, 2) k_fold_g2_sb_split_q(const G2A* __restrict__ hi, const G2A* __restrict__ pow , uint32_t half, SbDigits dg, G2J* __restrict__ parts , uint8_t* __restrict__ flag ) {
+    __shared__ uint4 park_[21 * 64];
+    const uint32_t i = blockIdx.x * blockDim.x + threadIdx.x;
+    if (i >= half) return;
+    const int t = blockIdx.y;
+    const size_t f = (size_t)t * half + i;
+    if (!((dg.mask >> t) & 1u)) { flag[f] = 0; return; }
+    flag[f] = fold_g2_split_lane_q(fold_g2_sb_src(hi, pow, half, t, i), t & 3, dg.d[t], dg.len, parts + f, park_);
+}
+__global__ void __launch_bounds__(64) k_fold_g2_sb_split_fix(const G2A* __restrict__ hi, const G2A* __restrict__ pow, uint32_t half, SbDigits dg, G2J* __restrict__ parts, const uint8_t* __restrict__ flag) {
+    for_flagged(flag, 16 * half, [&](uint32_t f) { const int t = (int)(f / half); const uint32_t i = f - (uint32_t)t * half; parts[f] = fold_g2_gls_split_complete(gls_image(*fold_g2_sb_src(hi, pow, half, t, i), t & 3), dg.d[t], dg.len); });
+}
+__global__ void __launch_bounds__(64) k_fold_g2_sb_combine(const G2J* __restrict__ parts, uint32_t mask, const G2A* __restrict__ lo, uint32_t half, G2J* __restrict__ out) {
+    const uint32_t i = blockIdx.x * blockDim.x + threadIdx.x;
+    if (i >= half) return;
+    G2J acc = to_jac(lo[i]);
+#pragma unroll 1
+    for (int t = 0; t < 16; ++t) if ((mask >> t) & 1u) acc = add(acc, parts[(size_t)t * half + i]);
+    out[i] = acc;
+}
+__global__ void __launch_bounds__(64, 2) k_pow2_steps_g2_q(const G2A* __restrict__ in, uint32_t n, int k, int steps, G2J* __restrict__ out ) {
+    const uint32_t i = blockIdx.x * blockDim.x + threadIdx.x;
+    if (i >= n) return;
+#if defined(__HIP_DEVICE_COMPILE__)
+    const G2A* bp = in + i;
+    bool inf; { const G2A b = *bp; inf = is_inf(b); }
+    if (inf) { for (int s = 0; s < steps; ++s) out[(size_t)s * n + i] = jac_inf<Fp2>(); return; }
+    JacQ2 d; j2_set(d, f2_from(opaque(bp)->x), f2_from(opaque(bp)->y), Fq2n{fq_one(), fq_zero()});
+    f2_pin(d.z);
+#pragma unroll 1
+    for (int s = 0; s < steps; ++s) {
+#pragma unroll 1
+        for (int t = 0; t < k; ++t) jdbl2_q(d);
+        out[(size_t)s * n + i] = G2J{f2_to(d.x), f2_to(d.y), f2_to(d.z)};
+    }
+#endif
 }
 
 __global__ void __launch_bounds__(64, 2) k_pow2_mul_g2_q(const G2A* __restrict__ in, uint32_t n, int k, G2J* __restrict__ out) {
```
